# rsjahnige/CRYSTALS-Kyber

Hardware: AMD Instinct MI355X
Metric: ML-KEM-768 encaps+decaps/sec at batch 2^20; achieved HBM GB/s vs peak (higher is better)
Workload: dtype u32+f32 (64-bit Keccak lanes as 2 x u32; mod-3329 arithmetic exact on integers < 2^24 in the fp32 pipe; u8/u16 I/O)

## Files before the change

### crystals-kyber_amd/csrc/mlkem_kernels.hpp

```cpp
#pragma once
#include "mlkem_device.hpp"

namespace mlkem {

constexpr int WAVE = 64;

#ifndef MLKEM_KECCAK_MINWAVES
#define MLKEM_KECCAK_MINWAVES 6
#endif

struct MsgView {
    const uint8_t* p0; size_t stride0; unsigned len0;
    const uint8_t* p1; size_t stride1; unsigned len1;
};

__device__ __forceinline__ uint2 load_qword_tail(const uint8_t* p, unsigned avail) {
    if (avail >= 8) return *reinterpret_cast<const uint2*>(p);
    uint2 v;
    v.x = 0; v.y = 0;
    for (unsigned i = 0; i < avail; i++) {
        const uint32_t b = p[i];
        if (i < 4) v.x |= b << (8 * i);
        else v.y |= b << (8 * (i - 4));
    }
    return v;
}

#ifndef MLKEM_STAGE_ROWS
#define MLKEM_STAGE_ROWS 32
#endif
#ifndef MLKEM_STAGE_DMA
#define MLKEM_STAGE_DMA 1
#endif
constexpr int STAGE_ROWS = MLKEM_STAGE_ROWS;
constexpr int STAGE_GROUP = MLKEM_STAGE_DMA ? 2 : 7;
constexpr int STAGE_PARTS = WAVE / STAGE_ROWS;

template <int RATE>
__device__ __forceinline__ void wave_stage_block(uint2* stage, const MsgView& mv, size_t item0, size_t n_items, unsigned voff,
                                                 int part) {
    constexpr int NQ = RATE / 8, TOT = STAGE_ROWS * NQ, ITERS = (TOT + WAVE - 1) / WAVE;
    const unsigned l = (unsigned)lane_id(), total = mv.len0 + mv.len1;
#pragma unroll 1
    for (int it0 = 0; it0 < ITERS; it0 += STAGE_GROUP)
#pragma unroll
    for (int it = it0; it < it0 + STAGE_GROUP; it++) {
        if (it >= ITERS) break;
        const unsigned f = (unsigned)it * WAVE + l;
        if (TOT % WAVE != 0 && f >= (unsigned)TOT) break;
        const unsigned row = f / NQ, col = f - row * NQ;
        size_t item = item0 + (size_t)(part * STAGE_ROWS) + row;
        if (item >= n_items) item = n_items - 1;
        const unsigned pos = voff + 8u * col;
        uint2 v;
        v.x = 0; v.y = 0;
        if (pos < total) {
            if (pos < mv.len0) v = load_qword_tail(mv.p0 + item * mv.stride0 + pos, mv.len0 - pos);
            else v = load_qword_tail(mv.p1 + item * mv.stride1 + (pos - mv.len0), total - pos);
        }
        stage[f] = v;
    }
}

template <int RATE>
__device__ __forceinline__ void lane_xor_row(KeccakState& s, const uint2* stage, int part) {
    constexpr int NQ = RATE / 8;
    const int l = lane_id();
    if (l / STAGE_ROWS == part) {
        const uint2* row = stage + (l % STAGE_ROWS) * NQ;
#pragma unroll
        for (int w = 0; w < NQ; w++) {
            const uint2 v = row[w];
            s.lo[w] ^= v.x;
            s.hi[w] ^= v.y;
        }
    }
}
template <int RATE>
__device__ __forceinline__ void wave_absorb_block(KeccakState& s, uint2* stage, const MsgView& mv, size_t item0, size_t n_items,
                                                  unsigned voff) {
#pragma unroll 1
    for (int part = 0; part < STAGE_PARTS; part++) {
        wave_stage_block<RATE>(stage, mv, item0, n_items, voff, part);
        wave_lds_fence();
        lane_xor_row<RATE>(s, stage, part);
        wave_lds_fence();
    }
}

#ifndef MLKEM_STAGE_DMA
#define MLKEM_STAGE_DMA 1
#endif
template <int RATE>
struct DmaStage {
    static constexpr int NW = RATE / 4;
    static constexpr int NJ = (NW + 3) / 4;
    static constexpr int DWORDS = 2 * NJ * WAVE;
};

template <int RATE>
__device__ __forceinline__ void wave_dma_half(uint32_t* stage, const MsgView& mv, size_t item0, unsigned voff, unsigned valid,
                                              int half) {
    using D = DmaStage<RATE>;
    const unsigned l = (unsigned)lane_id_fresh(), rr = l >> 2, c4 = 4u * (l & 3u);
    const unsigned off0 = rr * (unsigned)mv.stride0 + c4, off1 = rr * (unsigned)mv.stride1 + c4;
    lds_dma_begin();
#pragma unroll
    for (int j = 0; j < D::NJ; j++) {
        const unsigned pos = 16u * (unsigned)j;
        const bool seg0 = voff + pos < mv.len0;
        const uint8_t* base = seg0 ? mv.p0 + (voff + pos) : mv.p1 + (voff + pos - mv.len0);
        const size_t stride = seg0 ? mv.stride0 : mv.stride1;
        const unsigned off = seg0 ? off0 : off1;
        if (pos + c4 < valid) {
#pragma unroll
            for (int g = 0; g < 2; g++)
                lds_dma_dword(base + (item0 + (size_t)(32 * half + 16 * g)) * stride, off, stage + (g * D::NJ + j) * WAVE);
        }
    }
}

template <int RATE, bool FULL>
__device__ __forceinline__ void lane_xor_dma(KeccakState& s, const uint32_t* stage, unsigned valid, int half) {
    using D = DmaStage<RATE>;
    const int l = lane_id_fresh();
    const uint32_t m = (l >> 5) == half ? 0xFFFFFFFFu : 0u;
    const uint32_t* row = stage + ((l >> 4) & 1) * (D::NJ * WAVE) + (l & 15) * 4;
#pragma unroll
    for (int j = 0; j < D::NJ; j++) {
        if (FULL || 16u * (unsigned)j < valid) {
            const uint4 v = *reinterpret_cast<const uint4*>(row + WAVE * j);
            const uint32_t d[4] = {v.x, v.y, v.z, v.w};
#pragma unroll
            for (int k = 0; k < 4; k++) {
                const int w = 4 * j + k;
                if (w < D::NW && (FULL || 4u * (unsigned)w < valid)) {
                    if (w & 1) s.hi[w >> 1] = __builtin_amdgcn_bitop3_b32(s.hi[w >> 1], d[k], m, 0x78);
                    else s.lo[w >> 1] = __builtin_amdgcn_bitop3_b32(s.lo[w >> 1], d[k], m, 0x78);
                }
            }
        }
    }
}
template <int NQ>
__device__ __forceinline__ void pin_state(KeccakState& s) {
#ifndef MLKEM_EMU
#pragma unroll
    for (int w = 0; w < NQ; w++) {
        asm volatile("" : "+v"(s.lo[w]));
        asm volatile("" : "+v"(s.hi[w]));
    }
#endif
}
template <int RATE, bool FULL>
__device__ __forceinline__ void wave_absorb_dma(KeccakState& s, uint32_t* st32, const MsgView& mv, size_t item0, unsigned voff,
                                                unsigned valid) {
    lds_dma_wait();
    wave_lds_fence();
    lane_xor_dma<RATE, FULL>(s, st32, valid, 0);
    pin_state<RATE / 8>(s);
    wave_lds_fence();
    wave_dma_half<RATE>(st32, mv, item0, voff, valid, 1);
    lds_dma_wait();
    wave_lds_fence();
    lane_xor_dma<RATE, FULL>(s, st32, valid, 1);
    pin_state<RATE / 8>(s);
    wave_lds_fence();
}

__device__ __forceinline__ void keccak_xor_byte_rt(KeccakState& s, unsigned pos, uint32_t byte) {
    const unsigned w = pos >> 2;
    const uint32_t v = byte << (8 * (pos & 3));
#define MLKEM_XB(W) keccak_word<W>(s) ^= (w == W) ? v : 0u;
    MLKEM_XB(0) MLKEM_XB(1) MLKEM_XB(2) MLKEM_XB(3) MLKEM_XB(4) MLKEM_XB(5) MLKEM_XB(6) MLKEM_XB(7)
    MLKEM_XB(8) MLKEM_XB(9) MLKEM_XB(10) MLKEM_XB(11) MLKEM_XB(12) MLKEM_XB(13) MLKEM_XB(14) MLKEM_XB(15)
    MLKEM_XB(16) MLKEM_XB(17) MLKEM_XB(18) MLKEM_XB(19) MLKEM_XB(20) MLKEM_XB(21) MLKEM_XB(22) MLKEM_XB(23)
    MLKEM_XB(24) MLKEM_XB(25) MLKEM_XB(26) MLKEM_XB(27) MLKEM_XB(28) MLKEM_XB(29) MLKEM_XB(30) MLKEM_XB(31)
    MLKEM_XB(32) MLKEM_XB(33) MLKEM_XB(34) MLKEM_XB(35) MLKEM_XB(36) MLKEM_XB(37) MLKEM_XB(38) MLKEM_XB(39)
    MLKEM_XB(40) MLKEM_XB(41)
#undef MLKEM_XB
}

template <int RATE, int SUFFIX>
__device__ __forceinline__ void wave_sponge_absorb(KeccakState& s, uint2* stage, const MsgView& mv, size_t item0,
                                                   size_t n_items) {
    const unsigned total = mv.len0 + mv.len1;
    keccak_zero(s);
#if MLKEM_STAGE_DMA
    if (item0 + WAVE <= n_items && total != 0 && total % 4 == 0 && (mv.len1 == 0 || mv.len0 % 16 == 0) &&
        mv.stride0 < (1u << 27) && mv.stride1 < (1u << 27)) {
        uint32_t* st32 = reinterpret_cast<uint32_t*>(stage);
        const unsigned nfull = total / (unsigned)RATE, rem = total - nfull * (unsigned)RATE;
        wave_dma_half<RATE>(st32, mv, item0, 0, nfull ? (unsigned)RATE : rem, 0);
#pragma unroll 1
        for (unsigned b = 0; b < nfull; b++) {
            wave_absorb_dma<RATE, true>(s, st32, mv, item0, b * RATE, RATE);
            if (b + 1 < nfull) wave_dma_half<RATE>(st32, mv, item0, (b + 1) * RATE, RATE, 0);
            else if (rem) wave_dma_half<RATE>(st32, mv, item0, nfull * RATE, rem, 0);
            keccak_f1600(s);
        }
        if (rem) wave_absorb_dma<RATE, false>(s, st32, mv, item0, nfull * RATE, rem);
        keccak_xor_byte_rt(s, rem, SUFFIX);
        keccak_xor_byte<RATE - 1>(s, 0x80);
        keccak_f1600(s);
        return;
    }
#endif
    unsigned voff = 0;
    while (total - voff >= (unsigned)RATE) {
        wave_absorb_block<RATE>(s, stage, mv, item0, n_items, voff);
        keccak_f1600(s);
        voff += RATE;
    }
    const unsigned rem = total - voff;
    if (rem) wave_absorb_block<RATE>(s, stage, mv, item0, n_items, voff);
    keccak_xor_byte_rt(s, rem, SUFFIX);
    keccak_xor_byte<RATE - 1>(s, 0x80);
    keccak_f1600(s);
}

constexpr int stage_qwords(int max_rate) {
    const int sync_q = STAGE_ROWS * (max_rate / 8);
    const int dma_q = MLKEM_STAGE_DMA ? 2 * ((max_rate / 4 + 3) / 4) * WAVE / 2 : 0;
    return sync_q > dma_q ? sync_q : dma_q;
}
constexpr int STAGE_QWORDS = stage_qwords(168);

__device__ __forceinline__ void store32(uint8_t* base, size_t stride, size_t item, const uint32_t (&w)[8]) {
    uint32_t* p = reinterpret_cast<uint32_t*>(base + item * stride);
#pragma unroll
    for (int i = 0; i < 8; i++) p[i] = w[i];
}
__device__ __forceinline__ void load32(const uint8_t* base, size_t stride, size_t item, uint32_t (&w)[8]) {
    const uint32_t* p = reinterpret_cast<const uint32_t*>(base + item * stride);
#pragma unroll
    for (int i = 0; i < 8; i++) w[i] = p[i];
}
#define MLKEM_STATE_WORDS8(s, FIRST, w)                                                             \
    {                                                                                               \
        w[0] = keccak_word<FIRST + 0>(s); w[1] = keccak_word<FIRST + 1>(s); w[2] = keccak_word<FIRST + 2>(s); \
        w[3] = keccak_word<FIRST + 3>(s); w[4] = keccak_word<FIRST + 4>(s); w[5] = keccak_word<FIRST + 5>(s); \
        w[6] = keccak_word<FIRST + 6>(s); w[7] = keccak_word<FIRST + 7>(s);                         \
    }
#define MLKEM_SET_WORDS8(s, FIRST, w)                                                               \
    {                                                                                               \
        keccak_word<FIRST + 0>(s) = w[0]; keccak_word<FIRST + 1>(s) = w[1]; keccak_word<FIRST + 2>(s) = w[2]; \
        keccak_word<FIRST + 3>(s) = w[3]; keccak_word<FIRST + 4>(s) = w[4]; keccak_word<FIRST + 5>(s) = w[5]; \
        keccak_word<FIRST + 6>(s) = w[6]; keccak_word<FIRST + 7>(s) = w[7];                         \
    }

__device__ __forceinline__ void lane_G64(KeccakState& s, const uint32_t (&x)[8], const uint32_t (&y)[8]) {
    keccak_zero(s);
    MLKEM_SET_WORDS8(s, 0, x)
    MLKEM_SET_WORDS8(s, 8, y)
    keccak_xor_byte<64>(s, 0x06);
    keccak_xor_byte<71>(s, 0x80);
    keccak_f1600(s);
}

template <int K>
__global__ void __launch_bounds__(WAVE, MLKEM_KECCAK_MINWAVES) k_hash_encaps(size_t n, const uint8_t* __restrict__ ek, const uint8_t* __restrict__ m,
                                                      uint8_t* __restrict__ Kout, uint8_t* __restrict__ r_ws) {
    __shared__ __attribute__((aligned(16))) uint2 stage[stage_qwords(136)];
    constexpr unsigned EK = 384 * K + 32;
    const size_t item0 = (size_t)blockIdx.x * WAVE, item = item0 + lane_id();
    KeccakState s;
    MsgView mv{ek, EK, EK, ek, EK, 0};
    wave_sponge_absorb<136, 0x06>(s, stage, mv, item0, n);
    uint32_t h[8], mm[8], w[8];
    MLKEM_STATE_WORDS8(s, 0, h)
    const size_t it = item < n ? item : n - 1;
    load32(m, 32, it, mm);
    lane_G64(s, mm, h);
    if (item < n) {
        MLKEM_STATE_WORDS8(s, 0, w)
        store32(Kout, 32, item, w);
        MLKEM_STATE_WORDS8(s, 8, w)
        store32(r_ws, 32, item, w);
    }
}

__global__ void __launch_bounds__(WAVE, MLKEM_KECCAK_MINWAVES) k_hash_g_shared(size_t n, const uint8_t* __restrict__ m, const uint8_t* __restrict__ h,
                                                                               uint8_t* __restrict__ Kout, uint8_t* __restrict__ r_ws) {
    const size_t item = (size_t)blockIdx.x * WAVE + lane_id();
    const size_t it = item < n ? item : n - 1;
    uint32_t mm[8], hh[8], w[8];
    load32(m, 32, it, mm);
    load32(h, 0, 0, hh);
    KeccakState s;
    lane_G64(s, mm, hh);
    if (item < n) {
        MLKEM_STATE_WORDS8(s, 0, w)
        store32(Kout, 32, item, w);
        MLKEM_STATE_WORDS8(s, 8, w)
        store32(r_ws, 32, item, w);
    }
}
__global__ void __launch_bounds__(256) k_status_fill(size_t n, const uint8_t* __restrict__ h_calc, const uint8_t* __restrict__ h_stored,
                                                     int32_t* __restrict__ status) {
    uint32_t diff = 0;
#pragma unroll
    for (int i = 0; i < 8; i++) diff |= reinterpret_cast<const uint32_t*>(h_calc)[i] ^ reinterpret_cast<const uint32_t*>(h_stored)[i];
    const int32_t v = diff ? -5 : 0;
    for (size_t i = (size_t)blockIdx.x * blockDim.x + threadIdx.x; i < n; i += (size_t)gridDim.x * blockDim.x) status[i] = v;
}
__global__ void __launch_bounds__(256) k_seed_split(size_t n, const uint4* __restrict__ seed, uint4* __restrict__ d, uint4* __restrict__ z) {
    const size_t g = (size_t)blockIdx.x * blockDim.x + threadIdx.x;
    if (g >= 4 * n) return;
    const size_t item = g >> 2;
    const unsigned part = (unsigned)(g & 3);
    const uint4 v = seed[g];
    if (part < 2) d[2 * item + part] = v;
    else z[2 * item + part - 2] = v;
}

template <int K, int CLEN, bool HASH_CHECK, int JRATE = 168>
__global__ void __launch_bounds__(WAVE, MLKEM_KECCAK_MINWAVES) k_hash_decaps(size_t n, const uint8_t* __restrict__ dk, const uint8_t* __restrict__ c,
                                                      const uint8_t* __restrict__ m_ws, uint8_t* __restrict__ Kp_ws,
                                                      uint8_t* __restrict__ r_ws, uint8_t* __restrict__ Kbar_ws,
                                                      int32_t* __restrict__ status, size_t dk_stride) {
    __shared__ __attribute__((aligned(16))) uint2 stage[STAGE_QWORDS];
    constexpr unsigned EK = 384 * K + 32;
    const size_t DK = dk_stride;
    const size_t nb = (n + WAVE - 1) / WAVE;
    const bool check_role = HASH_CHECK && blockIdx.x < nb;
    const size_t item0 = (size_t)(HASH_CHECK && !check_role ? blockIdx.x - nb : blockIdx.x) * WAVE;
    KeccakState s;
    uint32_t h[8], w[8];
    auto my_item = [&]() {
        const size_t i2 = item0 + (size_t)lane_id_fresh();
        return i2 < n ? i2 : n - 1;
    };
    if (check_role) {
        MsgView mv{dk + 384 * K, DK, EK, dk, DK, 0};
        wave_sponge_absorb<136, 0x06>(s, stage, mv, item0, n);
        MLKEM_STATE_WORDS8(s, 0, w)
        load32(dk + 768 * K + 32, DK, my_item(), h);
        uint32_t diff = 0;
#pragma unroll
        for (int i = 0; i < 8; i++) diff |= w[i] ^ h[i];
        const size_t i2 = item0 + (size_t)lane_id_fresh();
        if (i2 < n && status) status[i2] = diff ? -5 : 0;
        return;
    }
    {
        MsgView mv{dk + 768 * K + 64, DK, 32, c, CLEN, CLEN};
        wave_sponge_absorb<JRATE, 0x1F>(s, stage, mv, item0, n);
        const size_t i2 = item0 + (size_t)lane_id_fresh();
        if (i2 < n) {
            MLKEM_STATE_WORDS8(s, 0, w)
            store32(Kbar_ws, 32, i2, w);
        }
    }
    uint32_t mm[8];
    const size_t it = my_item();
    load32(m_ws, 32, it, mm);
    load32(dk + 768 * K + 32, DK, it, h);
    lane_G64(s, mm, h);
    const size_t item = item0 + (size_t)lane_id_fresh();
    if (item < n) {
        MLKEM_STATE_WORDS8(s, 0, w)
        store32(Kp_ws, 32, item, w);
        MLKEM_STATE_WORDS8(s, 8, w)
        store32(r_ws, 32, item, w);
        if (!HASH_CHECK && status) status[item] = 0;
    }
}

template <int K>
__global__ void __launch_bounds__(WAVE, MLKEM_KECCAK_MINWAVES) k_hash_keygen_seed(size_t n, const uint8_t* __restrict__ d, uint8_t* __restrict__ rho_ws,
                                                           uint8_t* __restrict__ sigma_ws) {
    const size_t item = (size_t)blockIdx.x * WAVE + lane_id();
    const size_t it = item < n ? item : n - 1;
    KeccakState s;
    uint32_t dd[8], w[8];
    load32(d, 32, it, dd);
    keccak_zero(s);
    MLKEM_SET_WORDS8(s, 0, dd)
    keccak_xor_byte<32>(s, (uint32_t)K);
    keccak_xor_byte<33>(s, 0x06);
    keccak_xor_byte<71>(s, 0x80);
    keccak_f1600(s);
    if (item < n) {
        MLKEM_STATE_WORDS8(s, 0, w)
        store32(rho_ws, 32, item, w);
        MLKEM_STATE_WORDS8(s, 8, w)
        store32(sigma_ws, 32, item, w);
    }
}

template <int K>
__global__ void __launch_bounds__(WAVE, MLKEM_KECCAK_MINWAVES) k_hash_keygen_fin(size_t n, const uint8_t* __restrict__ ek, const uint8_t* __restrict__ z,
                                                          uint8_t* __restrict__ dk) {
    __shared__ __attribute__((aligned(16))) uint2 stage[stage_qwords(136)];
    constexpr unsigned EK = 384 * K + 32, DK = 768 * K + 96;
    const size_t item0 = (size_t)blockIdx.x * WAVE, item = item0 + lane_id();
    KeccakState s;
    MsgView mv{ek, EK, EK, ek, EK, 0};
    wave_sponge_absorb<136, 0x06>(s, stage, mv, item0, n);
    if (item < n) {
        uint32_t w[8];
        MLKEM_STATE_WORDS8(s, 0, w)
        store32(dk + 768 * K + 32, DK, item, w);
        load32(z, 32, item, w);
        store32(dk + 768 * K + 64, DK, item, w);
    }
}

template <int KIND>
__global__ void __launch_bounds__(WAVE, 4) k_hash_batch(size_t n, const uint8_t* __restrict__ msg, unsigned len,
                                                                            size_t stride, uint8_t* __restrict__ out) {
    constexpr int RATE = KIND == 0 ? 136 : KIND == 1 ? 72 : 168;
    __shared__ __attribute__((aligned(16))) uint2 stage[stage_qwords(RATE)];
    const size_t item0 = (size_t)blockIdx.x * WAVE;
    KeccakState s;
    MsgView mv{msg, stride, len, msg, stride, 0};
    uint32_t w[8];
    wave_sponge_absorb<RATE, KIND == 2 ? 0x1F : 0x06>(s, stage, mv, item0, n);
    const size_t item = item0 + (size_t)lane_id_fresh();
    if (item < n) {
        MLKEM_STATE_WORDS8(s, 0, w)
        store32(out, KIND == 1 ? 64 : 32, item, w);
        if (KIND == 1) {
            MLKEM_STATE_WORDS8(s, 8, w)
            store32(out + 32, 64, item, w);
        }
    }
}

template <int RATE>
__global__ void __launch_bounds__(WAVE) k_sponge_raw(size_t n, const uint8_t* __restrict__ msg, unsigned nblocks, uint8_t* __restrict__ out,
                                                     unsigned outlen, size_t out_stride) {
    __shared__ __attribute__((aligned(16))) uint2 stage[STAGE_QWORDS];
    const size_t item0 = (size_t)blockIdx.x * WAVE, item = item0 + lane_id();
    KeccakState s;
    const unsigned total = nblocks * RATE;
    MsgView mv{msg, total, total, msg, total, 0};
    keccak_zero(s);
    for (unsigned voff = 0; voff < total; voff += RATE) {
        wave_absorb_block<RATE>(s, stage, mv, item0, n, voff);
        keccak_f1600(s);
    }
    uint8_t* o = out + (item < n ? item : n - 1) * out_stride;
    for (unsigned done = 0; done < outlen; done += RATE) {
        if (done) keccak_f1600(s);
        const unsigned take = outlen - done < (unsigned)RATE ? outlen - done : (unsigned)RATE;
        if (item < n) {
#define MLKEM_SQ(W)                                                                                         \
            if constexpr (W < RATE / 4) {                                                                   \
                if (4u * W + 4u <= take) *reinterpret_cast<uint32_t*>(o + done + 4 * W) = keccak_word<W>(s); \
                else if (4u * W < take) {                                                                   \
                    const uint32_t v = keccak_word<W>(s);                                                   \
                    for (unsigned b = 0; 4u * W + b < take; b++) o[done + 4 * W + b] = (uint8_t)(v >> (8 * b)); \
                }                                                                                           \
            }
            MLKEM_SQ(0) MLKEM_SQ(1) MLKEM_SQ(2) MLKEM_SQ(3) MLKEM_SQ(4) MLKEM_SQ(5) MLKEM_SQ(6) MLKEM_SQ(7)
            MLKEM_SQ(8) MLKEM_SQ(9) MLKEM_SQ(10) MLKEM_SQ(11) MLKEM_SQ(12) MLKEM_SQ(13) MLKEM_SQ(14) MLKEM_SQ(15)
            MLKEM_SQ(16) MLKEM_SQ(17) MLKEM_SQ(18) MLKEM_SQ(19) MLKEM_SQ(20) MLKEM_SQ(21) MLKEM_SQ(22) MLKEM_SQ(23)
            MLKEM_SQ(24) MLKEM_SQ(25) MLKEM_SQ(26) MLKEM_SQ(27) MLKEM_SQ(28) MLKEM_SQ(29) MLKEM_SQ(30) MLKEM_SQ(31)
            MLKEM_SQ(32) MLKEM_SQ(33) MLKEM_SQ(34) MLKEM_SQ(35) MLKEM_SQ(36) MLKEM_SQ(37) MLKEM_SQ(38) MLKEM_SQ(39)
            MLKEM_SQ(40) MLKEM_SQ(41)
#undef MLKEM_SQ
        }
    }
}

constexpr int RING = 128;
constexpr int RING_STRIDE = RING + 8;

constexpr int RESUME_WORDS = 52;
struct SampleArgs {
    size_t n_xof;
    const uint8_t* rho;
    size_t rho_stride;
    int K;
    int transpose;
    uint16_t* A;
    unsigned xof_blocks;
    size_t n_prf;
    const uint8_t* r;
    int per_item;
    int n_eta1;
    int eta1;
    uint8_t* prf;
    unsigned prf_stride;
    uint32_t* leftover;
    uint32_t* resume;
    uint32_t resume_cap;
    int list_mode;
    int prf_rate;
    uint8_t* retries;
};

template <class OutFn>
__device__ __forceinline__ void prf_eta3_tail(KeccakState& s, unsigned rate, OutFn out_of_lane, bool mine) {
    const unsigned nw = rate / 4;
    if (mine) {
        uint32_t* out = out_of_lane();
#define MLKEM_PT(W) if (W < nw) out[W] = keccak_word<W>(s);
        MLKEM_PT(32) MLKEM_PT(33) MLKEM_PT(34) MLKEM_PT(35) MLKEM_PT(36) MLKEM_PT(37) MLKEM_PT(38) MLKEM_PT(39) MLKEM_PT(40) MLKEM_PT(41)
#undef MLKEM_PT
    }
    keccak_f1600(s);
    if (mine) {
        uint32_t* out = out_of_lane() + nw;
#define MLKEM_PT(W) if (nw + W < 48u) out[W] = keccak_word<W>(s);
        MLKEM_PT(0) MLKEM_PT(1) MLKEM_PT(2) MLKEM_PT(3) MLKEM_PT(4) MLKEM_PT(5) MLKEM_PT(6) MLKEM_PT(7)
        MLKEM_PT(8) MLKEM_PT(9) MLKEM_PT(10) MLKEM_PT(11) MLKEM_PT(12) MLKEM_PT(13)
#undef MLKEM_PT
    }
}

__device__ __forceinline__ void ring_flush(const int16_t* ring, uint16_t* A, size_t g, bool valid, int cnt, int& flushed) {
    const int l = lane_id();
    const int has = (cnt - flushed >= 64) && valid;
    if (__ballot(has) == 0) return;
    const int grp = l >> 3, sub = l & 7;
#pragma unroll 1
    for (int step = 0; step < 8; step++) {
        const int p = step * 8 + grp;
        const int p_has = __shfl(has, p);
        const int p_flushed = __shfl(flushed, p);
        const size_t gp = (size_t)(uint32_t)__shfl((int)(uint32_t)g, p);
        if (p_has) {
            const int16_t* src = ring + p * RING_STRIDE + (p_flushed & (RING - 1)) + sub * 8;
            uint4 v = *reinterpret_cast<const uint4*>(src);
            *reinterpret_cast<uint4*>(A + gp * 256 + p_flushed + sub * 8) = v;
        }
    }
    if (has) flushed += 64;
}

constexpr int SAMPLE_CAP = 278;
constexpr int sample_nt5(int cap, int g) { return cap - 224 - 4 * g >= 4 ? 4 : (cap - 224 - 4 * g <= 0 ? 0 : cap - 224 - 4 * g); }

#define MLKEM_CAND(d)                                                      \
    {                                                                      \
        const bool ok = ((d) < (unsigned)QB) && (cnt < 256);               \
        if (ok) myring[cnt & (RING - 1)] = (int16_t)(d);                   \
        cnt += ok ? 1 : 0;                                                 \
    }
#define MLKEM_GROUP4(W0, NT)                                                                      \
    {                                                                                             \
        const uint32_t w0 = keccak_word<W0>(s), w1 = keccak_word<W0 + 1>(s), w2 = keccak_word<W0 + 2>(s); \
        const uint32_t v0 = w0 & 0xFFFFFFu, v1 = (w0 >> 24) | ((w1 & 0xFFFFu) << 8);              \
        const uint32_t v2 = (w1 >> 16) | ((w2 & 0xFFu) << 16), v3 = w2 >> 8;                      \
        if (NT > 0) { MLKEM_CAND(v0 & 0xFFFu) MLKEM_CAND(v0 >> 12) }                              \
        if (NT > 1) { MLKEM_CAND(v1 & 0xFFFu) MLKEM_CAND(v1 >> 12) }                              \
        if (NT > 2) { MLKEM_CAND(v2 & 0xFFFu) MLKEM_CAND(v2 >> 12) }                              \
        if (NT > 3) { MLKEM_CAND(v3 & 0xFFFu) MLKEM_CAND(v3 >> 12) }                              \
    }
#define MLKEM_GROUP4_CAP(W0, G)                                                                   \
    if constexpr (sample_nt5(CAP, G) == 4) { MLKEM_GROUP4(W0, 4) }                                \
    else { if (blk == 4) MLKEM_GROUP4(W0, sample_nt5(CAP, G)) else MLKEM_GROUP4(W0, 4) }

template <int QB = KQ, int CAP = SAMPLE_CAP>
__global__ void __launch_bounds__(WAVE) k_sample(SampleArgs a) {
    __shared__ __attribute__((aligned(16))) int16_t ring[WAVE * RING_STRIDE];
    const int l = lane_id();
    KeccakState s;
    if (blockIdx.x < a.xof_blocks) {
        const size_t limit = a.list_mode ? (size_t)a.leftover[0] : a.n_xof;
        const size_t stride = a.list_mode ? (size_t)gridDim.x * WAVE : ~(size_t)0 / 2;
      for (size_t base = (size_t)blockIdx.x * WAVE; base < limit; base += stride) {
        const size_t slot = base + l;
        const bool valid = slot < limit;
        const size_t slot_c = valid ? slot : limit - 1;
        const size_t g = a.list_mode ? (size_t)a.leftover[2 + slot_c] : slot_c;
        const size_t gc = g;
        uint32_t seed[8];
        unsigned i0, i1;
        if (a.K) {
            const size_t kk = (size_t)(a.K * a.K), item = gc / kk;
            const unsigned e = (unsigned)(gc - item * kk), ra = e / (unsigned)a.K, cb = e - ra * (unsigned)a.K;
            load32(a.rho, a.rho_stride, item, seed);
            i0 = a.transpose ? ra : cb;
            i1 = a.transpose ? cb : ra;
        } else {
            const uint8_t* sp = a.rho + gc * a.rho_stride;
#pragma unroll
            for (int i = 0; i < 8; i++)
                seed[i] = (uint32_t)sp[4 * i] | ((uint32_t)sp[4 * i + 1] << 8) | ((uint32_t)sp[4 * i + 2] << 16) |
                          ((uint32_t)sp[4 * i + 3] << 24);
            i0 = sp[32];
            i1 = sp[33];
        }
        int16_t* myring = ring + l * RING_STRIDE;
        unsigned nretry = 0;
        int cnt = 0, flushed = 0;
        bool fresh = true;
        int blk = 0;
        while (true) {
            if (fresh) {
                keccak_zero(s);
                MLKEM_SET_WORDS8(s, 0, seed)
                keccak_xor_byte<32>(s, i0 & 0xFFu);
                keccak_xor_byte<33>(s, i1 & 0xFFu);
                keccak_xor_byte<34>(s, 0x1F);
                keccak_xor_byte<167>(s, 0x80);
                cnt = 0; flushed = 0; blk = 0; fresh = false;
            }
            keccak_f1600(s);
            MLKEM_GROUP4_CAP(0, 0) MLKEM_GROUP4_CAP(3, 1) MLKEM_GROUP4_CAP(6, 2) MLKEM_GROUP4_CAP(9, 3)
            MLKEM_GROUP4_CAP(12, 4) MLKEM_GROUP4_CAP(15, 5) MLKEM_GROUP4_CAP(18, 6)
            wave_lds_fence();
            ring_flush(ring, a.A, g, valid, cnt, flushed);
            wave_lds_fence();
            MLKEM_GROUP4_CAP(21, 7) MLKEM_GROUP4_CAP(24, 8) MLKEM_GROUP4_CAP(27, 9) MLKEM_GROUP4_CAP(30, 10)
            MLKEM_GROUP4_CAP(33, 11) MLKEM_GROUP4_CAP(36, 12) MLKEM_GROUP4_CAP(39, 13)
            wave_lds_fence();
            ring_flush(ring, a.A, g, valid, cnt, flushed);
            wave_lds_fence();
            blk++;
            if (blk == 5 && cnt < 256) {
                i0 = (i0 + 1) & 0xFFu;
                i1 = (i1 + 1) & 0xFFu;
                fresh = true;
                nretry++;
            }
            if (__ballot(cnt < 256) == 0) break;
        }
        if (a.retries && valid && !a.list_mode) a.retries[g] = (uint8_t)(nretry < 255u ? nretry : 255u);
        wave_lds_fence();
      }
    } else {
        const size_t g = (size_t)(blockIdx.x - a.xof_blocks) * WAVE + l;
        const size_t gc = g < a.n_prf ? g : a.n_prf - 1;
        uint32_t seed[8];
        unsigned ctr, eta;
        if (a.per_item) {
            const size_t item = gc / (size_t)a.per_item;
            ctr = (unsigned)(gc - item * (size_t)a.per_item);
            load32(a.r, 32, item, seed);
            eta = (int)ctr < a.n_eta1 ? (unsigned)a.eta1 : 2u;
        } else {
            const uint8_t* sp = a.r + gc * 33;
#pragma unroll
            for (int i = 0; i < 8; i++)
                seed[i] = (uint32_t)sp[4 * i] | ((uint32_t)sp[4 * i + 1] << 8) | ((uint32_t)sp[4 * i + 2] << 16) |
                          ((uint32_t)sp[4 * i + 3] << 24);
            ctr = sp[32];
            eta = (unsigned)a.eta1;
        }
        keccak_zero(s);
        MLKEM_SET_WORDS8(s, 0, seed)
        keccak_xor_byte<32>(s, ctr & 0xFFu);
        keccak_xor_byte<33>(s, 0x1F);
        if (a.prf_rate == 136) keccak_xor_byte<135>(s, 0x80);
        else keccak_xor_byte<167>(s, 0x80);
        keccak_f1600(s);
        uint32_t* out = reinterpret_cast<uint32_t*>(a.prf + gc * a.prf_stride);
        if (g < a.n_prf) {
#define MLKEM_OW(W) out[W] = keccak_word<W>(s);
            MLKEM_OW(0) MLKEM_OW(1) MLKEM_OW(2) MLKEM_OW(3) MLKEM_OW(4) MLKEM_OW(5) MLKEM_OW(6) MLKEM_OW(7)
            MLKEM_OW(8) MLKEM_OW(9) MLKEM_OW(10) MLKEM_OW(11) MLKEM_OW(12) MLKEM_OW(13) MLKEM_OW(14) MLKEM_OW(15)
            MLKEM_OW(16) MLKEM_OW(17) MLKEM_OW(18) MLKEM_OW(19) MLKEM_OW(20) MLKEM_OW(21) MLKEM_OW(22) MLKEM_OW(23)
            MLKEM_OW(24) MLKEM_OW(25) MLKEM_OW(26) MLKEM_OW(27) MLKEM_OW(28) MLKEM_OW(29) MLKEM_OW(30) MLKEM_OW(31)
        }
#undef MLKEM_OW
        if (__ballot(eta == 3) != 0) {
            const bool mine = g < a.n_prf && eta == 3;
            auto out_fn = [out]() { return out; };
            prf_eta3_tail(s, a.prf_rate == 136 ? 136u : 168u, out_fn, mine);
        }
    }
}

}
```

### crystals-kyber_amd/csrc/mlkem_keyset.hpp

```cpp
#pragma once
#include "mlkem_pipeline.hpp"

namespace mlkem {

constexpr int32_t KS_ERR_ARG = -101;

struct KeysetView {
    const uint8_t* keys = nullptr;
    size_t key_stride = 0;
    size_t ek_off = 0;
    const uint8_t* h = nullptr;
    const uint16_t* At = nullptr;
    size_t n_keys = 0;
    bool has_dk = false;
};

struct KeysetLimits {
    size_t enc_max_k[3] = {1536, 1024, 768}, dec_max_k[3] = {3072, 2048, 3072};
    size_t enc_lat_k[3] = {256, 512, 256}, dec_lat_k[3] = {384, 256, 256};
    size_t enc_max(int k) const { return enc_max_k[k - 2]; }
    size_t dec_max(int k) const { return dec_max_k[k - 2]; }
    size_t enc_lat(int k) const { return enc_lat_k[k - 2]; }
    size_t dec_lat(int k) const { return dec_lat_k[k - 2]; }
    void set_all(size_t max_items, size_t lat_items) {
        for (int i = 0; i < 3; i++) {
            if (max_items != (size_t)-1) enc_max_k[i] = dec_max_k[i] = max_items;
            if (lat_items != (size_t)-1) enc_lat_k[i] = dec_lat_k[i] = lat_items;
        }
    }
};

__device__ __forceinline__ size_t keyset_key(const uint32_t* __restrict__ idx, size_t n_keys, size_t item) {
    if (!idx) return 0;
    const size_t k = idx[item];
    return k < n_keys ? k : 0;
}

__global__ void __launch_bounds__(WAVE, MLKEM_KECCAK_MINWAVES) k_hash_g_keyset(size_t n, const uint32_t* __restrict__ idx, size_t n_keys,
                                                                               const uint8_t* __restrict__ m, const uint8_t* __restrict__ hs,
                                                                               uint8_t* __restrict__ Kout, uint8_t* __restrict__ r_ws) {
    const size_t item = (size_t)blockIdx.x * WAVE + lane_id();
    const size_t it = item < n ? item : n - 1;
    uint32_t mm[8], hh[8], w[8];
    load32(m, 32, it, mm);
    load32(hs, 32, keyset_key(idx, n_keys, it), hh);
    KeccakState s;
    lane_G64(s, mm, hh);
    if (item < n) {
        MLKEM_STATE_WORDS8(s, 0, w)
        store32(Kout, 32, item, w);
        MLKEM_STATE_WORDS8(s, 8, w)
        store32(r_ws, 32, item, w);
    }
}

__global__ void __launch_bounds__(256) k_keyset_gather32(size_t n, const uint32_t* __restrict__ idx, size_t n_keys, const uint8_t* __restrict__ src,
                                                         size_t stride, uint32_t* __restrict__ dst) {
    const size_t g = (size_t)blockIdx.x * blockDim.x + threadIdx.x;
    if (g >= 8 * n) return;
    const size_t item = g >> 3;
    dst[g] = reinterpret_cast<const uint32_t*>(src + keyset_key(idx, n_keys, item) * stride)[g & 7];
}

template <int K, int CLEN, int JRATE>
__global__ void __launch_bounds__(WAVE, MLKEM_KECCAK_MINWAVES) k_hash_decaps_keyset(size_t n, const uint32_t* __restrict__ idx, size_t n_keys,
                                                                                    const uint8_t* __restrict__ hs, uint8_t* __restrict__ z_ws,
                                                                                    const uint8_t* __restrict__ c, const uint8_t* __restrict__ m_ws,
                                                                                    uint8_t* __restrict__ Kp_ws, uint8_t* __restrict__ r_ws,
                                                                                    uint8_t* __restrict__ Kbar_ws) {
    __shared__ __attribute__((aligned(16))) uint2 stage[STAGE_QWORDS];
    const size_t item0 = (size_t)blockIdx.x * WAVE;
    KeccakState s;
    uint32_t h[8], w[8];
    {
        MsgView mv{z_ws, 32, 32, c, CLEN, CLEN};
        wave_sponge_absorb<JRATE, 0x1F>(s, stage, mv, item0, n);
        const size_t i2 = item0 + (size_t)lane_id_fresh();
        if (i2 < n) {
            MLKEM_STATE_WORDS8(s, 0, w)
            store32(Kbar_ws, 32, i2, w);
            uint32_t* zr = reinterpret_cast<uint32_t*>(z_ws + i2 * 32);
#pragma unroll
            for (int q = 0; q < 8; q++) zr[q] = 0u;
        }
    }
    uint32_t mm[8];
    const size_t i3 = item0 + (size_t)lane_id_fresh(), it = i3 < n ? i3 : n - 1;
    load32(m_ws, 32, it, mm);
    load32(hs, 32, keyset_key(idx, n_keys, it), h);
    lane_G64(s, mm, h);
    const size_t item = item0 + (size_t)lane_id_fresh();
    if (item < n) {
        MLKEM_STATE_WORDS8(s, 0, w)
        store32(Kp_ws, 32, item, w);
        MLKEM_STATE_WORDS8(s, 8, w)
        store32(r_ws, 32, item, w);
    }
}

template <int K, int ETA1, int DU, int DV, bool COMPARE>
__global__ void __launch_bounds__(WAVE * KPKE2_WAVES, kpke2_minwaves(K))
k_encrypt2_keyset(size_t n, const uint32_t* __restrict__ idx, size_t n_keys, const uint8_t* __restrict__ ek, size_t ek_stride,
                  const uint16_t* __restrict__ At, const uint8_t* __restrict__ msg, const uint8_t* __restrict__ prf, uint8_t* __restrict__ c_out,
                  const uint8_t* __restrict__ c_in, const uint8_t* __restrict__ Kp, const uint8_t* __restrict__ Kbar, uint8_t* __restrict__ Kout) {
    __shared__ K2Lds<K + 1> lds_all[KPKE2_WAVES];
    const int wv = wave_id();
    const size_t item0 = 2 * ((size_t)blockIdx.x * KPKE2_WAVES + wv);
    if (item0 >= n) return;
    const size_t h = (size_t)(lane_id() >> 5), item = item0 + h < n ? item0 + h : item0;
    const size_t key = keyset_key(idx, n_keys, item);
    encrypt2_body<K, ETA1, DU, DV, COMPARE>(lds_all[wv].xch, item0, n, ek + key * ek_stride, 0, msg, At + key * (size_t)(K * K * 256), prf,
                                            c_out, c_in, Kp, Kbar, Kout, (int32_t*)nullptr, 0);
}

template <int K, int DU, int DV>
__global__ void __launch_bounds__(64 * KPKE4_WAVES, kpke4_minwaves(K)) k_decrypt4_keyset(size_t n, const uint32_t* __restrict__ idx, size_t n_keys,
                                                                                       const uint8_t* __restrict__ dk, size_t dk_stride,
                                                                                       const uint8_t* __restrict__ c, uint8_t* __restrict__ m_out) {
    const size_t quad = (size_t)blockIdx.x * KPKE4_WAVES + wave_id();
    if (4 * quad >= n) return;
    const size_t item_raw = 4 * quad + (size_t)rntt_lane().p, item = item_raw < n ? item_raw : n - 1;
    decrypt4_body<K, DU, DV>(quad, n, dk + keyset_key(idx, n_keys, item) * dk_stride, 0, c, m_out);
}

__global__ void __launch_bounds__(256) k_keyset_fix(size_t n, const uint32_t* __restrict__ idx, size_t n_keys, uint8_t* __restrict__ c,
                                                    unsigned c_len, uint8_t* __restrict__ Kout, int32_t* __restrict__ status) {
    for (size_t i = (size_t)blockIdx.x * blockDim.x + threadIdx.x; i < n; i += (size_t)gridDim.x * blockDim.x) {
        const bool bad = idx && (size_t)idx[i] >= n_keys;
        if (status) status[i] = bad ? KS_ERR_ARG : 0;
        if (!bad) continue;
        uint32_t* k = reinterpret_cast<uint32_t*>(Kout + i * 32);
        for (int w = 0; w < 8; w++) k[w] = 0;
        if (c) {
            uint32_t* cw = reinterpret_cast<uint32_t*>(c + i * c_len);
            for (unsigned w = 0; w < c_len / 4; w++) cw[w] = 0;
        }
    }
}

__global__ void __launch_bounds__(256) k_keyset_status_or(size_t n, const int32_t* __restrict__ status, uint32_t* __restrict__ out) {
    uint32_t v = 0;
    for (size_t i = (size_t)blockIdx.x * blockDim.x + threadIdx.x; i < n; i += (size_t)gridDim.x * blockDim.x) v |= (uint32_t)status[i];
    if (v) atomicOr(out, v);
}

template <int K, int ETA1>
struct __attribute__((aligned(16))) KeysetHand {
    uint8_t prf[(2 * K + 1) * (ETA1 == 3 ? 192 : 128)];
    uint8_t r[32], m[32], Kp[32], Kbar[32];
};

__device__ __forceinline__ void keyset_small_reject(size_t item, uint8_t* c, unsigned c_len, uint8_t* Kout, int32_t* status) {
    const unsigned l = (unsigned)lane_id();
    if (l < 8) reinterpret_cast<uint32_t*>(Kout + item * 32)[l] = 0;
    if (c)
        for (unsigned w = l; w < c_len / 4; w += WAVE) reinterpret_cast<uint32_t*>(c + item * c_len)[w] = 0;
    if (l == 0 && status) status[item] = KS_ERR_ARG;
}

template <int K, int ETA1, int DU, int DV, int NW>
__global__ void __launch_bounds__(WAVE * NW)
k_encaps_keyset_small(size_t n, const uint32_t* __restrict__ idx, size_t n_keys, const uint8_t* __restrict__ ek, size_t ek_stride,
                      const uint8_t* __restrict__ hs, const uint16_t* __restrict__ At, const uint8_t* __restrict__ m, uint8_t* __restrict__ c,
                      uint8_t* __restrict__ Kout, int32_t* __restrict__ status, int prf_rate) {
    __shared__ K2Lds<K + 1> xl;
    __shared__ KeysetHand<K, ETA1> hand;
    __shared__ uint2 rc_tables[NW][WK_RC_ENTRIES];
    __shared__ SmallSync sy;
    constexpr unsigned CLEN = 32 * (DU * K + DV);
    const int wv = wave_id();
    const size_t item = blockIdx.x;
    if (item >= n) return;
    const size_t key = idx ? (size_t)idx[item] : 0;
    if (key >= n_keys) {
        if (wv == 0) keyset_small_reject(item, c, CLEN, Kout, status);
        return;
    }
    const uint8_t* my_ek = ek + key * ek_stride;
    WkLane cst;
    wk_lane_init(cst, rc_tables[wave_id()]);
    if (threadIdx.x == 0) { sy.next_job = K * K; sy.jobs_done = 0; sy.r_ready = 0; sy.kbar_ready = 0; }
    block_barrier();
    if (wv == 0) {
        const int i = wk_index();
        uint2 v;
        v.x = 0; v.y = 0;
        if (i >= 0 && i < 4) v = reinterpret_cast<const uint2*>(m + item * 32)[i];
        else if (i >= 4 && i < 8) v = reinterpret_cast<const uint2*>(hs + key * 32)[i - 4];
        WkState a;
        a.lo = v.x; a.hi = v.y;
        if (i == 8) { a.lo = 0x06u; a.hi = 0x80000000u; }
        wk_permute(a, cst);
        uint2 o;
        o.x = a.lo; o.y = a.hi;
        if (wk_primary() && i < 4) reinterpret_cast<uint2*>(Kout + item * 32)[i] = o;
        else if (wk_primary() && i < 8) reinterpret_cast<uint2*>(hand.r)[i - 4] = o;
        flag_signal(&sy.r_ready);
    }
    small_jobs<K, ETA1>(sy, cst, nullptr, true, nullptr, hand.r, hand.prf, 2 * K + 1, (unsigned)prf_rate, nullptr);
    if (wv != 0) return;
    flag_wait(&sy.jobs_done, (uint32_t)(2 * K + 1));
    encrypt1_body<K, ETA1, DU, DV, false>(xl.xch, my_ek, m + item * 32, At + key * (size_t)(K * K * 256), hand.prf, c + item * CLEN, nullptr,
                                          nullptr, nullptr, nullptr, nullptr);
    if (lane_id() == 0 && status) status[item] = 0;
    wave_lds_fence();
    wave_zero_lds(hand);
    wave_zero_lds(xl);
#ifdef MLKEM_EMU_LDS_PROBE
    if (lane_id() == 0) { MLKEM_EMU_LDS_PROBE(&hand, sizeof hand); MLKEM_EMU_LDS_PROBE(&xl, sizeof xl); }
#endif
}

template <int K, int ETA1, int DU, int DV, int JRATE, int NW>
__global__ void __launch_bounds__(WAVE * NW)
k_decaps_keyset_small(size_t n, const uint32_t* __restrict__ idx, size_t n_keys, const uint8_t* __restrict__ dk, size_t dk_stride,
                      const uint8_t* __restrict__ hs, const uint16_t* __restrict__ At, const uint8_t* __restrict__ c, uint8_t* __restrict__ Kout,
                      int32_t* __restrict__ status, int prf_rate) {
    static_assert(NW >= 2, "roles of waves 0 and 1");
    __shared__ K2Lds<K + 1> xl;
    __shared__ KeysetHand<K, ETA1> hand;
    __shared__ uint2 rc_tables[NW][WK_RC_ENTRIES];
    __shared__ SmallSync sy;
    constexpr unsigned DK = 768 * K + 96, CLEN = 32 * (DU * K + DV);
    const int wv = wave_id();
    const size_t item = blockIdx.x;
    if (item >= n) return;
    const size_t key = idx ? (size_t)idx[item] : 0;
    if (key >= n_keys) {
        if (wv == 0) keyset_small_reject(item, nullptr, CLEN, Kout, status);
        return;
    }
    const uint8_t* my_dk = dk + key * dk_stride;
    const uint8_t* my_c = c + item * CLEN;
    WkLane cst;
    wk_lane_init(cst, rc_tables[wave_id()]);
    const int i = wk_index();
    const bool prim = wk_primary();
    if (threadIdx.x == 0) { sy.next_job = K * K; sy.jobs_done = 0; sy.r_ready = 0; sy.kbar_ready = 0; }
    block_barrier();
    if (wv == 0) {
        decrypt4_body<K, DU, DV>(0, 1, my_dk, (size_t)DK, my_c, hand.m);
        wave_global_fence();
        uint2 v;
        v.x = 0; v.y = 0;
        if (i >= 0 && i < 4) v = reinterpret_cast<const uint2*>(hand.m)[i];
        else if (i >= 4 && i < 8) v = reinterpret_cast<const uint2*>(hs + key * 32)[i - 4];
        WkState a;
        a.lo = v.x; a.hi = v.y;
        if (i == 8) { a.lo = 0x06u; a.hi = 0x80000000u; }
        wk_permute(a, cst);
        uint2 o;
        o.x = a.lo; o.y = a.hi;
        if (prim && i < 4) reinterpret_cast<uint2*>(hand.Kp)[i] = o;
        else if (prim && i < 8) reinterpret_cast<uint2*>(hand.r)[i - 4] = o;
        flag_signal(&sy.r_ready);
    } else if (wv == 1) {
        WkState a;
        wk_absorb<JRATE, 0x1F>(a, cst, my_dk + 768 * K + 64, 32, my_c, 32 + CLEN);
        uint2 o;
        o.x = a.lo; o.y = a.hi;
        if (prim && i < 4) reinterpret_cast<uint2*>(hand.Kbar)[i] = o;
        flag_signal(&sy.kbar_ready);
    }
    small_jobs<K, ETA1>(sy, cst, nullptr, true, nullptr, hand.r, hand.prf, 2 * K + 1, (unsigned)prf_rate, nullptr);
    if (wv != 0) return;
    flag_wait(&sy.jobs_done, (uint32_t)(2 * K + 1));
    encrypt1_body<K, ETA1, DU, DV, true>(xl.xch, my_dk + 384 * K, hand.m, At + key * (size_t)(K * K * 256), hand.prf, nullptr, my_c, hand.Kp,
                                         hand.Kbar, Kout + item * 32, nullptr, &sy.kbar_ready);
    if (lane_id() == 0 && status) status[item] = 0;
    wave_lds_fence();
    wave_zero_lds(hand);
    wave_zero_lds(xl);
#ifdef MLKEM_EMU_LDS_PROBE
    if (lane_id() == 0) { MLKEM_EMU_LDS_PROBE(&hand, sizeof hand); MLKEM_EMU_LDS_PROBE(&xl, sizeof xl); }
#endif
}

inline size_t keyset_table_bytes_per_key(const ParamSet& p, bool has_dk) {
    return (has_dk ? (size_t)p.dk_len : (size_t)p.ek_len) + 32 + (size_t)(p.k * p.k) * 512;
}

template <int K>
inline void keyset_import_run(stream_t st, const ParamSet& p, const KeysetView& ks, uint8_t* hs, uint16_t* At, int32_t* status,
                              uint32_t* status_or, const Workspace& ws) {
    const size_t n = ks.n_keys;
    zero_u32x2(st, status_or);
    if (status) {
        const uint8_t* ek = ks.has_dk ? nullptr : ks.keys;
        const uint8_t* dk = ks.has_dk ? ks.keys : nullptr;
        check_keys_dispatch(st, p.set, n, ek, dk, nullptr, nullptr, status, nullptr, min_sz(n, ws.cap), ws);
        launch("k_keyset_status_or", k_keyset_status_or, min_sz(ceil_div(n, 256), 1024), 256u, st, n, (const int32_t*)status, status_or);
    }
    hash_launch(st, 0, n, ks.keys + ks.ek_off, p.ek_len, ks.key_stride, hs);
    for (size_t c0 = 0; c0 < n; c0 += ws.cap) {
        const size_t cn = min_sz(ws.cap, n - c0);
        Workspace w = ws;
        w.A = At + c0 * (size_t)(K * K * 256);
        launch_sample_split(st, p, cn, 0, ks.keys + c0 * ks.key_stride + ks.ek_off + 384 * K, ks.key_stride, 1, nullptr, 0, 0, w);
    }
}

inline void keyset_seed_run(stream_t st, const ParamSet& p, size_t n, const uint8_t* seed, uint8_t* dk, uint8_t* tmp, const Workspace& ws) {
    uint8_t *d = tmp, *z = d + n * 32, *ek = z + n * 32;
    launch("k_seed_split", k_seed_split, ceil_div(4 * n, 256), 256, st, n, reinterpret_cast<const uint4*>(seed), reinterpret_cast<uint4*>(d),
           reinterpret_cast<uint4*>(z));
    keygen_dispatch(st, p.set, n, d, z, ek, dk, ws);
}

template <int K, int ETA1, int DU, int DV>
inline void encaps_keyset_run(stream_t st, const ParamSet& p, const KeysetView& ks, size_t n, const uint32_t* idx, const uint8_t* m, uint8_t* c,
                              uint8_t* Kout, int32_t* status, const Workspace& ws, const KeysetLimits& lim) {
    if (n == 0) return;
    const uint8_t* ek = ks.keys + ks.ek_off;
    if (n <= lim.enc_max(K)) {
        const int rate = ws.fips ? 136 : 168;
        if (n <= lim.enc_lat(K))
            launch("k_encaps_keyset_small", k_encaps_keyset_small<K, ETA1, DU, DV, SMALL_WAVES>, n, WAVE * SMALL_WAVES, st, n, idx, ks.n_keys, ek,
                   ks.key_stride, ks.h, ks.At, m, c, Kout, status, rate);
        else
            launch("k_encaps_keyset_small", k_encaps_keyset_small<K, ETA1, DU, DV, SMALL_WAVES_DENSE>, n, WAVE * SMALL_WAVES_DENSE, st, n, idx,
                   ks.n_keys, ek, ks.key_stride, ks.h, ks.At, m, c, Kout, status, rate);
        return;
    }
    for (size_t h0 = 0; h0 < n; h0 += ws.hcap) {
        const size_t hn = min_sz(ws.hcap, n - h0);
        const uint32_t* idh = idx ? idx + h0 : nullptr;
        launch("k_hash_g_keyset", k_hash_g_keyset, ceil_div(hn, WAVE), WAVE, st, hn, idh, ks.n_keys, m + h0 * 32, ks.h, Kout + h0 * 32, ws.r);
        for (size_t c0 = 0; c0 < hn; c0 += ws.cap) {
            const size_t cn = min_sz(ws.cap, hn - c0), i0 = h0 + c0;
            launch_sample_split(st, p, 0, cn, nullptr, 0, 1, ws.r + c0 * 32, 2 * K + 1, K, ws);
            launch("k_encrypt_keyset", k_encrypt2_keyset<K, ETA1, DU, DV, false>, ceil_div(ceil_div(cn, 2), KPKE2_WAVES), WAVE * KPKE2_WAVES, st, cn,
                   idx ? idx + i0 : nullptr, ks.n_keys, ek, ks.key_stride, ks.At, m + i0 * 32, (const uint8_t*)ws.prf, c + i0 * p.c_len,
                   (const uint8_t*)nullptr, (const uint8_t*)nullptr, (const uint8_t*)nullptr, (uint8_t*)nullptr);
        }
    }
    if (idx || status)
        launch("k_keyset_fix", k_keyset_fix, min_sz(ceil_div(n, 256), 1024), 256u, st, n, idx, ks.n_keys, c, p.c_len, Kout, status);
}

template <int K, int ETA1, int DU, int DV>
inline void decaps_keyset_run(stream_t st, const ParamSet& p, const KeysetView& ks, size_t n, const uint32_t* idx, const uint8_t* c,
                              uint8_t* Kout, int32_t* status, const Workspace& ws, const KeysetLimits& lim) {
    constexpr int CLEN = 32 * (DU * K + DV);
    if (n == 0) return;
    if (n <= lim.dec_max(K)) {
        const int rate = ws.fips ? 136 : 168;
#define MLKEM_DKS(JR, NW) launch("k_decaps_keyset_small", k_decaps_keyset_small<K, ETA1, DU, DV, JR, NW>, n, WAVE * NW, st, n, idx, ks.n_keys, \
                                 ks.keys, ks.key_stride, ks.h, ks.At, c, Kout, status, rate)
        if (!ws.fips && n <= lim.dec_lat(K)) MLKEM_DKS(168, SMALL_WAVES);
        else if (!ws.fips) MLKEM_DKS(168, SMALL_WAVES_DENSE);
        else if (n <= lim.dec_lat(K)) MLKEM_DKS(136, SMALL_WAVES);
        else MLKEM_DKS(136, SMALL_WAVES_DENSE);
#undef MLKEM_DKS
        return;
    }
    for (size_t h0 = 0; h0 < n; h0 += ws.hcap) {
        const size_t hn = min_sz(ws.hcap, n - h0);
        const uint32_t* idh = idx ? idx + h0 : nullptr;
        const uint8_t* ch = c + h0 * p.c_len;
        launch("k_decrypt_keyset", k_decrypt4_keyset<K, DU, DV>, ceil_div(ceil_div(hn, 4), KPKE4_WAVES), 64 * KPKE4_WAVES, st, hn, idh, ks.n_keys,
               ks.keys, ks.key_stride, ch, ws.m);
        launch("k_keyset_gather32", k_keyset_gather32, ceil_div(8 * hn, 256), 256u, st, hn, idh, ks.n_keys, ks.keys + 768 * K + 64, ks.key_stride,
               reinterpret_cast<uint32_t*>(ws.rho));
        if (!ws.fips)
            launch("k_hash_decaps_keyset", k_hash_decaps_keyset<K, CLEN, 168>, ceil_div(hn, WAVE), WAVE, st, hn, idh, ks.n_keys, ks.h,
                   ws.rho, ch, (const uint8_t*)ws.m, ws.Kp, ws.r, ws.Kbar);
        else
            launch("k_hash_decaps_keyset", k_hash_decaps_keyset<K, CLEN, 136>, ceil_div(hn, WAVE), WAVE, st, hn, idh, ks.n_keys, ks.h,
                   ws.rho, ch, (const uint8_t*)ws.m, ws.Kp, ws.r, ws.Kbar);
        for (size_t c0 = 0; c0 < hn; c0 += ws.cap) {
            const size_t cn = min_sz(ws.cap, hn - c0), i0 = h0 + c0;
            launch_sample_split(st, p, 0, cn, nullptr, 0, 1, ws.r + c0 * 32, 2 * K + 1, K, ws);
            launch("k_encrypt_cmp_keyset", k_encrypt2_keyset<K, ETA1, DU, DV, true>, ceil_div(ceil_div(cn, 2), KPKE2_WAVES), WAVE * KPKE2_WAVES, st,
                   cn, idx ? idx + i0 : nullptr, ks.n_keys, ks.keys + 384 * K, ks.key_stride, ks.At, (const uint8_t*)(ws.m + c0 * 32),
                   (const uint8_t*)ws.prf, (uint8_t*)nullptr, c + i0 * p.c_len, (const uint8_t*)(ws.Kp + c0 * 32), (const uint8_t*)(ws.Kbar + c0 * 32),
                   Kout + i0 * 32);
        }
    }
    if (idx || status)
        launch("k_keyset_fix", k_keyset_fix, min_sz(ceil_div(n, 256), 1024), 256u, st, n, idx, ks.n_keys, (uint8_t*)nullptr, p.c_len, Kout, status);
}

inline int keyset_import_dispatch(stream_t st, const ParamSet& p, const KeysetView& ks, uint8_t* hs, uint16_t* At, int32_t* status,
                                  uint32_t* status_or, const Workspace& ws) {
    switch (p.set) {
    case 512: keyset_import_run<2>(st, p, ks, hs, At, status, status_or, ws); break;
    case 768: keyset_import_run<3>(st, p, ks, hs, At, status, status_or, ws); break;
    default: keyset_import_run<4>(st, p, ks, hs, At, status, status_or, ws); break;
    }
    return 0;
}
inline int encaps_keyset_dispatch(stream_t st, const ParamSet& p, const KeysetView& ks, size_t n, const uint32_t* idx, const uint8_t* m,
                                  uint8_t* c, uint8_t* K, int32_t* status, const Workspace& ws, const KeysetLimits& lim) {
    switch (p.set) {
    case 512: encaps_keyset_run<2, 3, 10, 4>(st, p, ks, n, idx, m, c, K, status, ws, lim); break;
    case 768: encaps_keyset_run<3, 2, 10, 4>(st, p, ks, n, idx, m, c, K, status, ws, lim); break;
    default: encaps_keyset_run<4, 2, 11, 5>(st, p, ks, n, idx, m, c, K, status, ws, lim); break;
    }
    return 0;
}
inline int decaps_keyset_dispatch(stream_t st, const ParamSet& p, const KeysetView& ks, size_t n, const uint32_t* idx, const uint8_t* c,
                                  uint8_t* K, int32_t* status, const Workspace& ws, const KeysetLimits& lim) {
    switch (p.set) {
    case 512: decaps_keyset_run<2, 3, 10, 4>(st, p, ks, n, idx, c, K, status, ws, lim); break;
    case 768: decaps_keyset_run<3, 2, 10, 4>(st, p, ks, n, idx, c, K, status, ws, lim); break;
    default: decaps_keyset_run<4, 2, 11, 5>(st, p, ks, n, idx, c, K, status, ws, lim); break;
    }
    return 0;
}

}
```

### crystals-kyber_amd/csrc/mlkem_kpke2.hpp

```cpp
#pragma once
#include "mlkem_arith.hpp"
#include "mlkem_rntt.hpp"
#include <type_traits>

namespace mlkem {

#ifndef MLKEM_KPKE2_WAVES
#define MLKEM_KPKE2_WAVES 1
#endif
constexpr int KPKE2_WAVES = MLKEM_KPKE2_WAVES;
#ifdef MLKEM_KPKE2_MINWAVES
constexpr int kpke2_minwaves(int) { return MLKEM_KPKE2_MINWAVES; }
#else
constexpr int kpke2_minwaves(int k) { return k == 2 ? 4 : k == 3 ? 3 : 2; }
#endif

template <int NP>
struct __attribute__((aligned(16))) K2Lds {
    float2 xch[NP][2][128];
};

__device__ __forceinline__ int k2_slot(int pair) { return pair ^ ((pair & 64) ? 0x15 : 0) ^ ((pair & 32) ? 0x0A : 0); }
enum K2Layout { K2_LA = 0, K2_LB = 1, K2_LC = 2, K2_NAT = 3 };
__device__ __forceinline__ int k2_blk(int t) { return (((t >> 2) & 3) << 3) | ((t >> 4) << 2) | (t & 3); }
__device__ __forceinline__ int k2_lc_hi(int t) { return (((t >> 2) & 3) << 2) | ((t >> 4) << 1) | ((t >> 1) & 1); }
template <int LAYOUT>
__device__ __forceinline__ int k2_pair(int t, int j) {
    if constexpr (LAYOUT == K2_LA) return (j << 5) | t;
    else if constexpr (LAYOUT == K2_LB) return ((t >> 3) << 5) | (j << 3) | (t & 7);
    else if constexpr (LAYOUT == K2_LC) return (k2_lc_hi(t) << 3) | (j << 1) | (t & 1);
    else return (k2_blk(t) << 2) | j;
}
template <int LAYOUT>
__device__ __forceinline__ void k2_write(float2* xh, int t, const v2f (&p)[4]) {
#pragma unroll
    for (int j = 0; j < 4; j++) {
        float2 v;
        v.x = p[j].x; v.y = p[j].y;
        xh[k2_slot(k2_pair<LAYOUT>(t, j))] = v;
    }
}
template <int LAYOUT>
__device__ __forceinline__ void k2_read(const float2* xh, int t, v2f (&p)[4]) {
#pragma unroll
    for (int j = 0; j < 4; j++) {
        const float2 v = xh[k2_slot(k2_pair<LAYOUT>(t, j))];
        p[j] = v2f{v.x, v.y};
    }
}
template <int FROM, int TO, int NP>
__device__ __forceinline__ void k2_exchange(float2 (*xch)[2][128], int h, int t, v2f (&p)[NP][4]) {
#pragma unroll
    for (int q = 0; q < NP; q++) k2_write<FROM>(xch[q][h], t, p[q]);
    wave_lds_fence();
#pragma unroll
    for (int q = 0; q < NP; q++) k2_read<TO>(xch[q][h], t, p[q]);
    wave_lds_fence();
}

struct K2Tw {
    Tw b0, b1, b2, c0, c1, c2, d0, d1;
};
__device__ __forceinline__ void k2_twiddles_fwd(K2Tw& w, int t) {
    const Tw* z = ZETA_F.z;
    const int b = t >> 3, c = k2_lc_hi(t), n = k2_blk(t);
    w.b0 = z[4 + b]; w.b1 = z[8 + 2 * b]; w.b2 = z[9 + 2 * b];
    w.c0 = z[16 + c]; w.c1 = z[32 + 2 * c]; w.c2 = z[33 + 2 * c];
    w.d0 = z[64 + 2 * n]; w.d1 = z[65 + 2 * n];
}
__device__ __forceinline__ void k2_twiddles_inv(K2Tw& w, int t) {
    const Tw* z = ZETA_F.z;
    const int b = t >> 3, c = k2_lc_hi(t), n = k2_blk(t);
    w.d0 = z[127 - 2 * n]; w.d1 = z[126 - 2 * n];
    w.c1 = z[63 - 2 * c]; w.c2 = z[62 - 2 * c]; w.c0 = z[31 - c];
    w.b1 = z[15 - 2 * b]; w.b2 = z[14 - 2 * b]; w.b0 = z[7 - b];
}

template <int N>
__device__ __forceinline__ void k2_shoup_n(const Tw (&z)[N], v2f (&b)[N]) {
    v2f km[N], nk[N];
#pragma unroll
    for (int i = 0; i < N; i++) km[i] = fma2(b[i], splat2(z[i].zq), splat2(F_MAGIC));
#pragma unroll
    for (int i = 0; i < N; i++) nk[i] = fma2(km[i], splat2(-F_Q), splat2(F_MAGIC_Q));
#pragma unroll
    for (int i = 0; i < N; i++) b[i] = fma2(b[i], splat2(z[i].z), nk[i]);
}
template <int N>
__device__ __forceinline__ void k2_fred_n(v2f (&x)[N]) {
    v2f k[N];
#pragma unroll
    for (int i = 0; i < N; i++) k[i] = fma2(x[i], splat2(F_INVQ), splat2(F_MAGIC));
#pragma unroll
    for (int i = 0; i < N; i++) k[i] = k[i] - splat2(F_MAGIC);
#pragma unroll
    for (int i = 0; i < N; i++) x[i] = fma2(k[i], splat2(-F_Q), x[i]);
}
template <int N, bool GS>
__device__ __forceinline__ void k2_bfly_n(v2f (&a)[N], v2f (&b)[N], const Tw (&z)[N]) {
    if constexpr (!GS) {
        k2_shoup_n<N>(z, b);
#pragma unroll
        for (int i = 0; i < N; i++) { const v2f tt = b[i]; b[i] = a[i] - tt; a[i] = a[i] + tt; }
    } else {
        v2f d[N];
#pragma unroll
        for (int i = 0; i < N; i++) d[i] = b[i] - a[i];
#pragma unroll
        for (int i = 0; i < N; i++) a[i] = a[i] + b[i];
        k2_shoup_n<N>(z, d);
#pragma unroll
        for (int i = 0; i < N; i++) b[i] = d[i];
    }
}
template <int NP, bool GS>
__device__ __forceinline__ void k2_layer_hi(v2f (&p)[NP][4], Tw z) {
    v2f a[2 * NP], b[2 * NP];
    Tw zz[2 * NP];
#pragma unroll
    for (int q = 0; q < NP; q++) { a[2 * q] = p[q][0]; b[2 * q] = p[q][2]; a[2 * q + 1] = p[q][1]; b[2 * q + 1] = p[q][3]; zz[2 * q] = z; zz[2 * q + 1] = z; }
    k2_bfly_n<2 * NP, GS>(a, b, zz);
#pragma unroll
    for (int q = 0; q < NP; q++) { p[q][0] = a[2 * q]; p[q][2] = b[2 * q]; p[q][1] = a[2 * q + 1]; p[q][3] = b[2 * q + 1]; }
}
template <int NP, bool GS>
__device__ __forceinline__ void k2_layer_lo(v2f (&p)[NP][4], Tw z01, Tw z23) {
    v2f a[2 * NP], b[2 * NP];
    Tw zz[2 * NP];
#pragma unroll
    for (int q = 0; q < NP; q++) { a[2 * q] = p[q][0]; b[2 * q] = p[q][1]; a[2 * q + 1] = p[q][2]; b[2 * q + 1] = p[q][3]; zz[2 * q] = z01; zz[2 * q + 1] = z23; }
    k2_bfly_n<2 * NP, GS>(a, b, zz);
#pragma unroll
    for (int q = 0; q < NP; q++) { p[q][0] = a[2 * q]; p[q][1] = b[2 * q]; p[q][2] = a[2 * q + 1]; p[q][3] = b[2 * q + 1]; }
}
template <int NP, int R0, int R1>
__device__ __forceinline__ void k2_fred_pairs(v2f (&p)[NP][4]) {
    v2f x[2 * NP];
#pragma unroll
    for (int q = 0; q < NP; q++) { x[2 * q] = p[q][R0]; x[2 * q + 1] = p[q][R1]; }
    k2_fred_n<2 * NP>(x);
#pragma unroll
    for (int q = 0; q < NP; q++) { p[q][R0] = x[2 * q]; p[q][R1] = x[2 * q + 1]; }
}

template <int NP>
__device__ __forceinline__ void k2_ntt(v2f (&p)[NP][4], float2 (*xch)[2][128], int h, int t, const K2Tw& w) {
    k2_layer_hi<NP, false>(p, FZ1);
    k2_layer_lo<NP, false>(p, FZ2, FZ3);
    k2_exchange<K2_LA, K2_LB, NP>(xch, h, t, p);
    k2_layer_hi<NP, false>(p, w.b0);
    k2_layer_lo<NP, false>(p, w.b1, w.b2);
    k2_exchange<K2_LB, K2_LC, NP>(xch, h, t, p);
    k2_layer_hi<NP, false>(p, w.c0);
    k2_layer_lo<NP, false>(p, w.c1, w.c2);
    k2_exchange<K2_LC, K2_NAT, NP>(xch, h, t, p);
    k2_layer_lo<NP, false>(p, w.d0, w.d1);
}
template <int NP>
__device__ __forceinline__ void k2_intt(v2f (&p)[NP][4], float2 (*xch)[2][128], int h, int t, const K2Tw& w) {
    k2_layer_lo<NP, true>(p, w.d0, w.d1);
    k2_fred_pairs<NP, 0, 2>(p);
    k2_exchange<K2_NAT, K2_LC, NP>(xch, h, t, p);
    k2_layer_lo<NP, true>(p, w.c1, w.c2);
    k2_layer_hi<NP, true>(p, w.c0);
    k2_fred_pairs<NP, 0, 1>(p);
    k2_exchange<K2_LC, K2_LB, NP>(xch, h, t, p);
    k2_layer_lo<NP, true>(p, w.b1, w.b2);
    k2_layer_hi<NP, true>(p, w.b0);
    k2_fred_pairs<NP, 0, 1>(p);
    k2_exchange<K2_LB, K2_LA, NP>(xch, h, t, p);
    k2_layer_lo<NP, true>(p, FZ3, FZ2);
    {
        v2f sm[2 * NP], df[2 * NP];
        Tw zs[2 * NP], zd[2 * NP];
#pragma unroll
        for (int q = 0; q < NP; q++)
#pragma unroll
            for (int m = 0; m < 2; m++) {
                sm[2 * q + m] = p[q][m] + p[q][m + 2];
                df[2 * q + m] = p[q][m + 2] - p[q][m];
                zs[2 * q + m] = F_INV128; zd[2 * q + m] = F_INV128_Z1;
            }
        k2_shoup_n<2 * NP>(zs, sm);
        k2_shoup_n<2 * NP>(zd, df);
#pragma unroll
        for (int q = 0; q < NP; q++)
#pragma unroll
            for (int m = 0; m < 2; m++) { p[q][m] = sm[2 * q + m]; p[q][m + 2] = df[2 * q + m]; }
    }
    k2_exchange<K2_LA, K2_NAT, NP>(xch, h, t, p);
}

template <int ETA>
struct K2CbdRaw {
    uint32_t w[ETA == 2 ? 1 : 2];
};
template <int ETA>
__device__ __forceinline__ void k2_cbd_load_la(const uint8_t* prf, int t, K2CbdRaw<ETA>& r) {
    if constexpr (ETA == 2) {
        r.w[0] = (uint32_t)prf[t] | ((uint32_t)prf[t + 32] << 8) | ((uint32_t)prf[t + 64] << 16) | ((uint32_t)prf[t + 96] << 24);
    } else {
        uint32_t f[4];
#pragma unroll
        for (int j = 0; j < 4; j++) {
            const int o = ((3 * t) >> 1) + 48 * j;
            f[j] = (((uint32_t)prf[o] | ((uint32_t)prf[o + 1] << 8)) >> (4 * (t & 1))) & 0xFFFu;
        }
        r.w[0] = f[0] | (f[1] << 12);
        r.w[1] = f[2] | (f[3] << 12);
    }
}
__device__ __forceinline__ uint32_t k2_cbd_load_nat2(const uint8_t* prf, int t) { return reinterpret_cast<const uint32_t*>(prf)[t]; }
template <bool BIASED = false>
__device__ __forceinline__ void k2_cbd2_eval8(uint32_t t, v2f (&p)[4]) {
    const uint32_t s = (t & 0x55555555u) + ((t >> 1) & 0x55555555u);
    const uint32_t d = ((s & 0x33333333u) + 0x22222222u) - ((s >> 2) & 0x33333333u);
    const uint32_t lo = d & 0x0F0F0F0Fu, hi = (d >> 4) & 0x0F0F0F0Fu;
    float fl[4] = {(float)(lo & 0xFFu), (float)((lo >> 8) & 0xFFu), (float)((lo >> 16) & 0xFFu), (float)(lo >> 24)};
    float fh[4] = {(float)(hi & 0xFFu), (float)((hi >> 8) & 0xFFu), (float)((hi >> 16) & 0xFFu), (float)(hi >> 24)};
#ifndef MLKEM_EMU
    asm volatile("" : "+v"(fl[0]), "+v"(fl[1]), "+v"(fl[2]), "+v"(fl[3]), "+v"(fh[0]), "+v"(fh[1]), "+v"(fh[2]), "+v"(fh[3]));
#endif
#pragma unroll
    for (int j = 0; j < 4; j++) {
        if constexpr (BIASED) p[j] = v2f{fl[j], fh[j]};
        else p[j] = v2f{fl[j], fh[j]} - splat2(2.0f);
    }
}
template <int ETA>
__device__ __forceinline__ void k2_cbd_eval(const K2CbdRaw<ETA>& r, v2f (&p)[4]) {
    if constexpr (ETA == 2) {
        k2_cbd2_eval8<false>(r.w[0], p);
    } else {
        float a[4], b[4];
        cbd_eval_f<3>(r.w[0], a);
        cbd_eval_f<3>(r.w[1], b);
        p[0] = v2f{a[0], a[1]}; p[1] = v2f{a[2], a[3]}; p[2] = v2f{b[0], b[1]}; p[3] = v2f{b[2], b[3]};
    }
}

__device__ __forceinline__ void k2_gamma(const v2f (&y)[4], Tw d0, Tw d1, float (&yg)[4]) {
    yg[0] = fmulmod_shoup(d0, y[0].y);
    yg[1] = fmulmod_shoup(tw_neg(d0), y[1].y);
    yg[2] = fmulmod_shoup(d1, y[2].y);
    yg[3] = fmulmod_shoup(tw_neg(d1), y[3].y);
}
__device__ __forceinline__ void k2_basemul_acc(v2f (&acc)[4], const v2f (&a)[4], const v2f (&y)[4], const float (&yg)[4]) {
    v2f c[4];
#pragma unroll
    for (int j = 0; j < 4; j++) c[j] = fma2(splat2(a[j].x), y[j], acc[j]);
#pragma unroll
    for (int j = 0; j < 4; j++) {
        c[j].x = __builtin_fmaf(a[j].y, yg[j], c[j].x);
        c[j].y = __builtin_fmaf(a[j].y, y[j].x, c[j].y);
    }
    k2_fred_n<4>(c);
#pragma unroll
    for (int j = 0; j < 4; j++) acc[j] = c[j];
}

__device__ __forceinline__ void k2_unpack16(const uint4 v, v2f (&p)[4]) {
    const uint32_t w[4] = {v.x, v.y, v.z, v.w};
#pragma unroll
    for (int j = 0; j < 4; j++) p[j] = v2f{(float)(w[j] & 0xFFFFu), (float)(w[j] >> 16)};
}
__device__ __forceinline__ void k2_decode12(uint32_t w0, uint32_t w1, uint32_t w2, v2f (&p)[4]) {
    const uint32_t c0 = w0 & 0xFFFu, c1 = (w0 >> 12) & 0xFFFu, c2 = __builtin_amdgcn_alignbit(w1, w0, 24) & 0xFFFu, c3 = (w1 >> 4) & 0xFFFu;
    const uint32_t c4 = (w1 >> 16) & 0xFFFu, c5 = __builtin_amdgcn_alignbit(w2, w1, 28) & 0xFFFu, c6 = (w2 >> 8) & 0xFFFu, c7 = w2 >> 20;
    p[0] = v2f{(float)c0, (float)c1}; p[1] = v2f{(float)c2, (float)c3}; p[2] = v2f{(float)c4, (float)c5}; p[3] = v2f{(float)c6, (float)c7};
}

__device__ __forceinline__ uint32_t f_bits(float x) {
    union { float f; uint32_t u; } v;
    v.f = x;
    return v.u;
}
template <int D, bool BIASED = false>
__device__ __forceinline__ void k2_compress4(const v2f (&x)[4], unsigned (&c)[8]) {
    v2f tt[4], k0m[4], k0[4], r[4], km[4];
#pragma unroll
    for (int j = 0; j < 4; j++) tt[j] = fma2(x[j], splat2((float)(1 << D)), splat2(BIASED ? -(float)(2 << D) : 0.0f));
#pragma unroll
    for (int j = 0; j < 4; j++) k0m[j] = fma2(tt[j], splat2(F_INVQ), splat2(F_MAGIC));
#pragma unroll
    for (int j = 0; j < 4; j++) k0[j] = k0m[j] - splat2(F_MAGIC);
#pragma unroll
    for (int j = 0; j < 4; j++) r[j] = fma2(k0[j], splat2(-F_Q), tt[j]);
#pragma unroll
    for (int j = 0; j < 4; j++) km[j] = fma2(r[j], splat2(F_INVQ), splat2(F_MAGIC));
#pragma unroll
    for (int j = 0; j < 4; j++) {
        c[2 * j] = (f_bits(k0m[j].x) + f_bits(km[j].x)) & ((1u << D) - 1u);
        c[2 * j + 1] = (f_bits(k0m[j].y) + f_bits(km[j].y)) & ((1u << D) - 1u);
    }
}

__device__ __forceinline__ uint32_t k2_swap1(uint32_t v) {
#ifdef MLKEM_EMU
    return (uint32_t)emu_quad_shfl((int)v, (int)((threadIdx.x & 3) ^ 1));
#else
    return (uint32_t)__builtin_amdgcn_mov_dpp((int)v, 0xB1, 0xF, 0xF, true);
#endif
}
__device__ __forceinline__ uint32_t k2_prev_in_quad(uint32_t v) {
#ifdef MLKEM_EMU
    const int l = (int)(threadIdx.x & 3);
    return (uint32_t)emu_quad_shfl((int)v, l ? l - 1 : l);
#else
    return (uint32_t)__builtin_amdgcn_mov_dpp((int)v, 0x90, 0xF, 0xF, true);
#endif
}
__device__ __forceinline__ uint32_t k2_shl_hi(uint32_t hi, uint32_t lo, unsigned s) {
    return s ? __builtin_amdgcn_alignbit(hi, lo, 32u - s) : hi;
}

template <int D>
struct K2Piece {
    static_assert(D == 4 || D == 5 || D == 10 || D == 11 || D == 12, "ciphertext / key encodings of ML-KEM");
    static constexpr int NW = D == 4 ? 1 : D == 5 ? 2 : 3;
    uint32_t w[NW];
    static __device__ __forceinline__ int first(int t) {
        if constexpr (D == 4) return t;
        else if constexpr (D == 12) return 3 * t;
        else if constexpr (D == 10) return 5 * (t >> 1) + ((t & 1) ? 3 : 0);
        else if constexpr (D == 11) return 11 * (t >> 2) + ((88 * (t & 3)) >> 5);
        else return 5 * (t >> 2) + (t & 3);
    }
    static __device__ __forceinline__ int count(int t) {
        if constexpr (D == 4) return 1;
        else if constexpr (D == 12) return 3;
        else if constexpr (D == 10) return (t & 1) ? 2 : 3;
        else if constexpr (D == 11) return (t & 3) ? 3 : 2;
        else return (t & 3) == 3 ? 2 : 1;
    }
};
template <int D>
__device__ __forceinline__ void k2_encode(const unsigned (&c)[8], int t, K2Piece<D>& o) {
    if constexpr (D == 4) {
        o.w[0] = c[0] | (c[1] << 4) | (c[2] << 8) | (c[3] << 12) | (c[4] << 16) | (c[5] << 20) | (c[6] << 24) | (c[7] << 28);
    } else if constexpr (D == 12) {
        o.w[0] = c[0] | (c[1] << 12) | (c[2] << 24);
        o.w[1] = (c[2] >> 8) | (c[3] << 4) | (c[4] << 16) | (c[5] << 28);
        o.w[2] = (c[5] >> 4) | (c[6] << 8) | (c[7] << 20);
    } else if constexpr (D == 10) {
        const uint32_t v0 = c[0] | (c[1] << 10) | (c[2] << 20) | (c[3] << 30);
        const uint32_t v1 = (c[3] >> 2) | (c[4] << 8) | (c[5] << 18) | (c[6] << 28);
        const uint32_t v2 = (c[6] >> 4) | (c[7] << 6);
        const uint32_t other0 = k2_swap1(v0);
        const unsigned sh = (t & 1) ? 16u : 0u;
        o.w[0] = __builtin_amdgcn_alignbit(v1, v0, sh);
        o.w[1] = __builtin_amdgcn_alignbit(v2, v1, sh);
        o.w[2] = v2 | (other0 << 16);
    } else if constexpr (D == 11) {
        const uint32_t v0 = c[0] | (c[1] << 11) | (c[2] << 22);
        const uint32_t v1 = (c[2] >> 10) | (c[3] << 1) | (c[4] << 12) | (c[5] << 23);
        const uint32_t v2 = (c[5] >> 9) | (c[6] << 2) | (c[7] << 13);
        const int j = t & 3;
        const unsigned sh = (88u * (unsigned)j) & 31u;
        const uint32_t e0 = v0 << sh, e1 = k2_shl_hi(v1, v0, sh), e2 = k2_shl_hi(v2, v1, sh), e3 = k2_shl_hi(0u, v2, sh);
        const uint32_t tail = j == 0 ? e2 : e3;
        const uint32_t prev = k2_prev_in_quad(tail);
        o.w[0] = e0 | (j ? prev : 0u);
        o.w[1] = e1;
        o.w[2] = e2;
    } else {
        const uint32_t v0 = c[0] | (c[1] << 5) | (c[2] << 10) | (c[3] << 15) | (c[4] << 20) | (c[5] << 25) | (c[6] << 30);
        const uint32_t v1 = (c[6] >> 2) | (c[7] << 3);
        const int j = t & 3;
        const unsigned sh = 8u * (unsigned)j;
        const uint32_t e0 = v0 << sh, e1 = k2_shl_hi(v1, v0, sh);
        const uint32_t prev = k2_prev_in_quad(e1);
        o.w[0] = e0 | (j ? prev : 0u);
        o.w[1] = e1;
    }
}
template <int D>
__device__ __forceinline__ void k2_piece_load(const uint8_t* poly, int t, K2Piece<D>& o) {
    const uint32_t* g = reinterpret_cast<const uint32_t*>(poly) + K2Piece<D>::first(t);
#pragma unroll
    for (int i = 0; i < K2Piece<D>::NW; i++) o.w[i] = i < K2Piece<D>::count(t) ? stream_load4(g + i) : 0u;
}
template <int D>
__device__ __forceinline__ void k2_piece_store(uint8_t* poly, int t, const K2Piece<D>& o) {
    uint32_t* g = reinterpret_cast<uint32_t*>(poly) + K2Piece<D>::first(t);
#pragma unroll
    for (int i = 0; i < K2Piece<D>::NW; i++)
        if (i < K2Piece<D>::count(t)) g[i] = o.w[i];
}
template <int D>
__device__ __forceinline__ uint32_t k2_piece_diff(int t, const K2Piece<D>& a, const K2Piece<D>& ref) {
    uint32_t d = 0;
#pragma unroll
    for (int i = 0; i < K2Piece<D>::NW; i++)
        if (i < K2Piece<D>::count(t)) d |= a.w[i] ^ ref.w[i];
    return d;
}
template <int D, bool COMPARE, bool BIASED = false>
__device__ __forceinline__ uint32_t k2_emit(const v2f (&p)[4], int t, uint8_t* out, const K2Piece<D>& ref, bool store) {
    unsigned c[8];
    k2_compress4<D, BIASED>(p, c);
    K2Piece<D> o;
    k2_encode<D>(c, t, o);
    if constexpr (COMPARE) return k2_piece_diff<D>(t, o, ref);
    if (store) k2_piece_store<D>(out, t, o);
    return 0;
}

template <int K, int ETA1, int DU, int DV, bool COMPARE>
__device__ __forceinline__ void
encrypt2_body(float2 (*xch)[2][128], size_t item0, size_t n, const uint8_t* __restrict__ ek, size_t ek_stride, const uint8_t* __restrict__ msg,
              const uint16_t* __restrict__ A, const uint8_t* __restrict__ prf, uint8_t* __restrict__ c_out, const uint8_t* __restrict__ c_in,
              const uint8_t* __restrict__ Kp, const uint8_t* __restrict__ Kbar, uint8_t* __restrict__ Kout, int32_t* __restrict__ mod_status,
              size_t a_stride) {
    const int l = lane_id(), h = l >> 5, t = l & 31, nb = k2_blk(t);
    const bool valid = item0 + (size_t)h < n;
    const unsigned hh = valid ? (unsigned)h : 0u;
    constexpr unsigned PS = (ETA1 == 3) ? 192 : 128, CLEN = 32 * (DU * K + DV), PRFLEN = (2 * K + 1) * PS;
    const uint8_t* my_prf = prf + item0 * (size_t)PRFLEN + (size_t)(hh * PRFLEN);
    const uint8_t* my_ek = ek + item0 * ek_stride + (size_t)(hh * (unsigned)ek_stride);
    const uint16_t* my_A = A + item0 * a_stride + (size_t)(hh * (unsigned)a_stride);
    uint8_t* my_c = COMPARE ? nullptr : c_out + item0 * CLEN + (size_t)(hh * CLEN);
    const uint8_t* my_cin = COMPARE ? c_in + item0 * CLEN + (size_t)(hh * CLEN) : nullptr;
    const size_t item = item0 + hh;

    K2CbdRaw<ETA1> raw_y[K];
#pragma unroll
    for (int b = 0; b < K; b++) k2_cbd_load_la<ETA1>(my_prf + b * PS, t, raw_y[b]);
    uint4 a_all[K + 1][K];
#pragma unroll
    for (int a = 0; a < K; a++)
#pragma unroll
        for (int b = 0; b < K; b++) a_all[a][b] = *reinterpret_cast<const uint4*>(my_A + (a * K + b) * 256 + 8 * nb);
#pragma unroll
    for (int b = 0; b < K; b++) {
        const uint32_t* gp = reinterpret_cast<const uint32_t*>(my_ek + 384 * b) + 3 * nb;
        a_all[K][b].x = stream_load4(gp); a_all[K][b].y = stream_load4(gp + 1); a_all[K][b].z = stream_load4(gp + 2); a_all[K][b].w = 0u;
    }
    uint32_t raw_e[K + 1];
#pragma unroll
    for (int a = 0; a <= K; a++) raw_e[a] = k2_cbd_load_nat2(my_prf + (K + a) * PS, nb);
    const unsigned mb = msg[item * 32 + nb];

    v2f yh[K][4];
    float yg[K][4];
    {
        K2Tw tw;
        k2_twiddles_fwd(tw, t);
#pragma unroll
        for (int b = 0; b < K; b++) k2_cbd_eval<ETA1>(raw_y[b], yh[b]);
        k2_ntt<K>(yh, xch, h, t, tw);
#pragma unroll
        for (int b = 0; b < K; b++) {
            k2_fred_n<4>(yh[b]);
            k2_gamma(yh[b], tw.d0, tw.d1, yg[b]);
        }
    }
    uint32_t diff = 0;
    bool over = false;
    constexpr int NG = K + 1;
    v2f acc[NG][4];
    K2Piece<DU> cu_ref[NG];
    K2Piece<DV> cv_ref;
#pragma unroll
    for (int a = 0; a < NG; a++) {
#pragma unroll
        for (int j = 0; j < 4; j++) acc[a][j] = splat2(0.f);
#pragma unroll
        for (int b = 0; b < K; b++) {
            v2f av[4];
            if (a < K) {
                k2_unpack16(a_all[a][b], av);
            } else {
                k2_decode12(a_all[a][b].x, a_all[a][b].y, a_all[a][b].z, av);
#pragma unroll
                for (int j = 0; j < 4; j++) over = over || (av[j].x >= F_Q) || (av[j].y >= F_Q);
            }
            k2_basemul_acc(acc[a], av, yh[b], yg[b]);
        }
    }
    if constexpr (COMPARE) {
#pragma unroll
        for (int a = 0; a < NG; a++) {
            if (a < K) k2_piece_load<DU>(my_cin + a * 32 * DU, nb, cu_ref[a]);
            else k2_piece_load<DV>(my_cin + K * 32 * DU, nb, cv_ref);
        }
    }
    {
        K2Tw twi;
        k2_twiddles_inv(twi, t);
        k2_intt<NG>(acc, xch, h, t, twi);
    }
#pragma unroll
    for (int a = 0; a < NG; a++) {
        v2f e[4];
        k2_cbd2_eval8<true>(raw_e[a], e);
#pragma unroll
        for (int j = 0; j < 4; j++) acc[a][j] = acc[a][j] + e[j];
        if (a < K) {
            diff |= k2_emit<DU, COMPARE, true>(acc[a], nb, COMPARE ? nullptr : my_c + a * 32 * DU, cu_ref[a], valid);
        } else {
#pragma unroll
            for (int j = 0; j < 4; j++)
                acc[a][j] = acc[a][j] + v2f{((mb >> (2 * j)) & 1u) ? 1665.0f : 0.0f, ((mb >> (2 * j + 1)) & 1u) ? 1665.0f : 0.0f};
            diff |= k2_emit<DV, COMPARE, true>(acc[a], nb, COMPARE ? nullptr : my_c + K * 32 * DU, cv_ref, valid);
        }
    }
    if (mod_status) {
        const unsigned long long bal = __ballot(over);
        const bool bad = ((bal >> (32 * h)) & 0xFFFFFFFFull) != 0;
        if (t == 0 && valid) mod_status[item] = bad ? -4 : 0;
    }
    if constexpr (COMPARE) {
        const unsigned long long bal = __ballot(diff != 0);
        const uint32_t reject = ((bal >> (32 * h)) & 0xFFFFFFFFull) != 0 ? 0xFFFFFFFFu : 0u;
        if (t < 8 && valid) {
            const uint32_t kp = reinterpret_cast<const uint32_t*>(Kp + item * 32)[t];
            const uint32_t kb = reinterpret_cast<const uint32_t*>(Kbar + item * 32)[t];
            reinterpret_cast<uint32_t*>(Kout + item * 32)[t] = (kp & ~reject) | (kb & reject);
        }
    }
}
template <int K, int ETA1, int DU, int DV, bool COMPARE, bool A_T = false>
__device__ __forceinline__ void
encrypt1_body(float2 (*xch)[2][128], const uint8_t* __restrict__ ek, const uint8_t* __restrict__ msg, const uint16_t* __restrict__ A,
              const uint8_t* __restrict__ prf, uint8_t* __restrict__ c_out, const uint8_t* __restrict__ c_in, const uint8_t* __restrict__ Kp,
              const uint8_t* Kbar, uint8_t* __restrict__ Kout, int32_t* __restrict__ mod_status,
              const uint32_t* kbar_flag = nullptr) {
    const int l = lane_id(), h = l >> 5, t = l & 31, nb = k2_blk(t);
    constexpr unsigned PS = (ETA1 == 3) ? 192 : 128;
    constexpr int NG = K + 1, NL = (NG + 1) / 2;
    auto kind = [](int i) constexpr { return 2 * i + 1 < K ? 0 : (2 * i < K ? 1 : 2); };

    K2CbdRaw<ETA1> raw_y[K];
#pragma unroll
    for (int b = 0; b < K; b++) k2_cbd_load_la<ETA1>(prf + b * PS, t, raw_y[b]);
    uint4 a_all[NL][K];
    uint32_t raw_e[NL];
#pragma unroll
    for (int i = 0; i < NL; i++) {
        const int a = kind(i) == 2 ? K : 2 * i + h;
        const bool is_v = kind(i) == 2 || (kind(i) == 1 && h == 1);
#pragma unroll
        for (int b = 0; b < K; b++) {
            if (is_v) {
                const uint32_t* gp = reinterpret_cast<const uint32_t*>(ek + 384 * b) + 3 * nb;
                a_all[i][b].x = gp[0]; a_all[i][b].y = gp[1]; a_all[i][b].z = gp[2]; a_all[i][b].w = 0u;
            } else {
                a_all[i][b] = *reinterpret_cast<const uint4*>(A + (A_T ? b * K + a : a * K + b) * 256 + 8 * nb);
            }
        }
        raw_e[i] = k2_cbd_load_nat2(prf + (K + a) * PS, nb);
    }
    const unsigned mb = msg[nb];

    v2f yh[K][4];
    float yg[K][4];
    {
        K2Tw tw;
        k2_twiddles_fwd(tw, t);
#pragma unroll
        for (int b = 0; b < K; b++) k2_cbd_eval<ETA1>(raw_y[b], yh[b]);
        k2_ntt<K>(yh, xch, h, t, tw);
#pragma unroll
        for (int b = 0; b < K; b++) {
            k2_fred_n<4>(yh[b]);
            k2_gamma(yh[b], tw.d0, tw.d1, yg[b]);
        }
    }
    uint32_t diff = 0;
    bool over = false;
    v2f acc[NL][4];
    K2Piece<DU> cu_ref[NL];
    K2Piece<DV> cv_ref;
#pragma unroll
    for (int i = 0; i < NL; i++) {
        const bool is_v = kind(i) == 2 || (kind(i) == 1 && h == 1);
#pragma unroll
        for (int j = 0; j < 4; j++) acc[i][j] = splat2(0.f);
#pragma unroll
        for (int b = 0; b < K; b++) {
            v2f av[4];
            if (is_v) {
                k2_decode12(a_all[i][b].x, a_all[i][b].y, a_all[i][b].z, av);
#pragma unroll
                for (int j = 0; j < 4; j++) over = over || (av[j].x >= F_Q) || (av[j].y >= F_Q);
            } else {
                k2_unpack16(a_all[i][b], av);
            }
            k2_basemul_acc(acc[i], av, yh[b], yg[b]);
        }
    }
    if constexpr (COMPARE) {
#pragma unroll
        for (int i = 0; i < NL; i++) {
            const int a = kind(i) == 2 ? K : 2 * i + h;
            const bool is_v = kind(i) == 2 || (kind(i) == 1 && h == 1);
            if (is_v) k2_piece_load<DV>(c_in + K * 32 * DU, nb, cv_ref);
            else k2_piece_load<DU>(c_in + a * 32 * DU, nb, cu_ref[i]);
        }
    }
    {
        K2Tw twi;
        k2_twiddles_inv(twi, t);
        k2_intt<NL>(acc, xch, h, t, twi);
    }
#pragma unroll
    for (int i = 0; i < NL; i++) {
        const int a = kind(i) == 2 ? K : 2 * i + h;
        const bool is_v = kind(i) == 2 || (kind(i) == 1 && h == 1);
        const bool store = kind(i) != 2 || h == 0;
        v2f e[4];
        k2_cbd2_eval8<true>(raw_e[i], e);
#pragma unroll
        for (int j = 0; j < 4; j++) acc[i][j] = acc[i][j] + e[j];
        if (is_v) {
#pragma unroll
            for (int j = 0; j < 4; j++)
                acc[i][j] = acc[i][j] + v2f{((mb >> (2 * j)) & 1u) ? 1665.0f : 0.0f, ((mb >> (2 * j + 1)) & 1u) ? 1665.0f : 0.0f};
            diff |= k2_emit<DV, COMPARE, true>(acc[i], nb, COMPARE ? nullptr : c_out + K * 32 * DU, cv_ref, store);
        } else {
            diff |= k2_emit<DU, COMPARE, true>(acc[i], nb, COMPARE ? nullptr : c_out + a * 32 * DU, cu_ref[i], store);
        }
    }
    if (mod_status) {
        const bool bad = __ballot(over) != 0;
        if (l == 0) mod_status[0] = bad ? -4 : 0;
    }
    if constexpr (COMPARE) {
        const uint32_t reject = __ballot(diff != 0) != 0 ? 0xFFFFFFFFu : 0u;
        if (kbar_flag) flag_wait(kbar_flag, 1u);
        if (l < 8) {
            const uint32_t kp = reinterpret_cast<const uint32_t*>(Kp)[l];
            const uint32_t kb = reinterpret_cast<const uint32_t*>(Kbar)[l];
            reinterpret_cast<uint32_t*>(Kout)[l] = (kp & ~reject) | (kb & reject);
        }
    }
}

template <int K, int ETA1, int DU, int DV, bool COMPARE>
__global__ void __launch_bounds__(WAVE * KPKE2_WAVES, kpke2_minwaves(K))
k_encrypt2(size_t n, const uint8_t* __restrict__ ek, size_t ek_stride, const uint8_t* __restrict__ msg, const uint16_t* __restrict__ A,
           const uint8_t* __restrict__ prf, uint8_t* __restrict__ c_out, const uint8_t* __restrict__ c_in, const uint8_t* __restrict__ Kp,
           const uint8_t* __restrict__ Kbar, uint8_t* __restrict__ Kout, int32_t* __restrict__ mod_status, size_t a_stride) {
    __shared__ K2Lds<K + 1> lds_all[KPKE2_WAVES];
    const int wv = wave_id();
    const size_t item0 = 2 * ((size_t)blockIdx.x * KPKE2_WAVES + wv);
    if (item0 >= n) return;
    encrypt2_body<K, ETA1, DU, DV, COMPARE>(lds_all[wv].xch, item0, n, ek, ek_stride, msg, A, prf, c_out, c_in, Kp, Kbar, Kout, mod_status, a_stride);
}

__device__ __forceinline__ void k2_canon(const v2f (&p)[4], unsigned (&c)[8]) {
    v2f r[4] = {p[0], p[1], p[2], p[3]};
    k2_fred_n<4>(r);
#pragma unroll
    for (int j = 0; j < 4; j++) {
        const int a = (int)r[j].x, b = (int)r[j].y;
        c[2 * j] = (unsigned)(a + ((a >> 31) & KQ));
        c[2 * j + 1] = (unsigned)(b + ((b >> 31) & KQ));
    }
}

template <int K, int ETA1, bool KEM_DK>
__device__ __forceinline__ void
keygen2_body(float2 (*xch)[2][128], size_t item0, size_t n, const uint16_t* __restrict__ A, const uint8_t* __restrict__ prf,
             const uint8_t* __restrict__ rho, uint8_t* __restrict__ ek, uint8_t* __restrict__ dk) {
    const int l = lane_id(), h = l >> 5, t = l & 31, nb = k2_blk(t);
    const bool valid = item0 + (size_t)h < n;
    const unsigned hh = valid ? (unsigned)h : 0u;
    constexpr unsigned PS = (ETA1 == 3) ? 192 : 128, EK = 384 * K + 32, DK = KEM_DK ? 768 * K + 96 : 384 * K, PRFLEN = 2 * K * PS;
    const uint8_t* my_prf = prf + item0 * (size_t)PRFLEN + (size_t)(hh * PRFLEN);
    const uint16_t* my_A = A + item0 * (size_t)(K * K * 256) + (size_t)(hh * (unsigned)(K * K * 256));
    uint8_t* my_ek = ek + item0 * EK + (size_t)(hh * EK);
    uint8_t* my_dk = dk + item0 * DK + (size_t)(hh * DK);
    const size_t item = item0 + hh;

    K2CbdRaw<ETA1> raw_s[K], raw_e[K];
#pragma unroll
    for (int b = 0; b < K; b++) k2_cbd_load_la<ETA1>(my_prf + b * PS, t, raw_s[b]);
    constexpr bool PF = K >= 3;
    uint4 a_all[K][K];
    if constexpr (PF) {
#pragma unroll
        for (int a = 0; a < K; a++)
#pragma unroll
            for (int b = 0; b < K; b++) a_all[a][b] = *reinterpret_cast<const uint4*>(my_A + (a * K + b) * 256 + 8 * nb);
    }
#pragma unroll
    for (int a = 0; a < K; a++) k2_cbd_load_la<ETA1>(my_prf + (K + a) * PS, t, raw_e[a]);
    const uint32_t rho_w = reinterpret_cast<const uint32_t*>(rho + item * 32)[t & 7];
    K2Tw tw;
    k2_twiddles_fwd(tw, t);
    v2f sh[K][4];
    float sg[K][4];
#pragma unroll
    for (int b = 0; b < K; b++) k2_cbd_eval<ETA1>(raw_s[b], sh[b]);
    k2_ntt<K>(sh, xch, h, t, tw);
#pragma unroll
    for (int b = 0; b < K; b++) {
        k2_fred_n<4>(sh[b]);
        k2_gamma(sh[b], tw.d0, tw.d1, sg[b]);
        unsigned c[8];
        k2_canon(sh[b], c);
        K2Piece<12> o;
        k2_encode<12>(c, nb, o);
        if (valid) k2_piece_store<12>(my_dk + 384 * b, nb, o);
    }
    v2f eh[K][4];
#pragma unroll
    for (int a = 0; a < K; a++) k2_cbd_eval<ETA1>(raw_e[a], eh[a]);
    k2_ntt<K>(eh, xch, h, t, tw);
#pragma unroll
    for (int a = 0; a < K; a++) {
        v2f acc[4] = {splat2(0.f), splat2(0.f), splat2(0.f), splat2(0.f)};
#pragma unroll
        for (int b = 0; b < K; b++) {
            v2f av[4];
            if constexpr (!PF) a_all[a][b] = *reinterpret_cast<const uint4*>(my_A + (a * K + b) * 256 + 8 * nb);
            k2_unpack16(a_all[a][b], av);
            k2_basemul_acc(acc, av, sh[b], sg[b]);
        }
#pragma unroll
        for (int j = 0; j < 4; j++) acc[j] = acc[j] + eh[a][j];
        unsigned c[8];
        k2_canon(acc, c);
        K2Piece<12> o;
        k2_encode<12>(c, nb, o);
        if (valid) {
            k2_piece_store<12>(my_ek + 384 * a, nb, o);
            if constexpr (KEM_DK) k2_piece_store<12>(my_dk + 384 * K + 384 * a, nb, o);
        }
    }
    if (t < 8 && valid) {
        reinterpret_cast<uint32_t*>(my_ek + 384 * K)[t] = rho_w;
        if constexpr (KEM_DK) reinterpret_cast<uint32_t*>(my_dk + 768 * K)[t] = rho_w;
    }
}
template <int K, int ETA1, bool KEM_DK>
__global__ void __launch_bounds__(WAVE * KPKE2_WAVES, K == 2 ? kpke2_minwaves(2) : kpke2_minwaves(K + 1))
k_keygen2(size_t n, const uint16_t* __restrict__ A, const uint8_t* __restrict__ prf, const uint8_t* __restrict__ rho,
          uint8_t* __restrict__ ek, uint8_t* __restrict__ dk) {
    __shared__ K2Lds<K> lds_all[KPKE2_WAVES];
    const int wv = wave_id();
    const size_t item0 = 2 * ((size_t)blockIdx.x * KPKE2_WAVES + wv);
    if (item0 >= n) return;
    keygen2_body<K, ETA1, KEM_DK>(lds_all[wv].xch, item0, n, A, prf, rho, ek, dk);
}

}
```

### crystals-kyber_amd/csrc/mlkem_pipeline.hpp

```cpp
#pragma once
#include "mlkem_kernels.hpp"
#include "mlkem_sampler.hpp"
#include "mlkem_arith.hpp"
#include "mlkem_rntt.hpp"
#include "mlkem_kpke4.hpp"
#include "mlkem_kpke2.hpp"
#include "mlkem_wkeccak.hpp"
#include "mlkem_small.hpp"
#include "mlkem_sha3r.hpp"
#include "mlkem_check.hpp"
#include <stdlib.h>
#ifndef MLKEM_EMU
#include <vector>
#endif

namespace mlkem {

#ifdef MLKEM_EMU
using stream_t = void*;
#else
using stream_t = hipStream_t;
#endif

#ifndef MLKEM_EMU
struct LaunchRecorder {
    struct Rec { const char* label; hipEvent_t a, b; };
    std::vector<Rec> recs;
    bool failed = false;
};
inline LaunchRecorder*& launch_recorder() {
    static thread_local LaunchRecorder* r = nullptr;
    return r;
}
#endif

template <class... KArgs, class... Args>
inline void launch(const char* label, void (*kfn)(KArgs...), size_t grid, unsigned block, stream_t st, Args... args) {
    if (grid == 0) return;
#ifdef MLKEM_EMU
    (void)st; (void)label;
    emu::launch((unsigned)grid, block, [=] { kfn(args...); });
#else
    LaunchRecorder* rec = launch_recorder();
    LaunchRecorder::Rec r{label, nullptr, nullptr};
    bool timed = rec && hipEventCreate(&r.a) == hipSuccess && hipEventCreate(&r.b) == hipSuccess && hipEventRecord(r.a, st) == hipSuccess;
    kfn<<<dim3((unsigned)grid), dim3(block), 0, st>>>(args...);
    if (timed) timed = hipEventRecord(r.b, st) == hipSuccess;
    if (timed) {
        rec->recs.push_back(r);
    } else if (rec) {
        rec->failed = true;
        if (r.a) (void)hipEventDestroy(r.a);
        if (r.b) (void)hipEventDestroy(r.b);
    }
#endif
}

inline void zero_u32x2(stream_t st, uint32_t* p) {
#ifdef MLKEM_EMU
    (void)st;
    p[0] = 0; p[1] = 0;
#else
    (void)hipMemsetAsync(p, 0, 2 * sizeof(uint32_t), st);
#endif
}

struct ParamSet {
    int set, k, eta1, eta2, du, dv;
    unsigned ek_len, dk_len, c_len;
};
inline bool param_set(int set, ParamSet& p) {
    switch (set) {
    case 512: p = {512, 2, 3, 2, 10, 4, 0, 0, 0}; break;
    case 768: p = {768, 3, 2, 2, 10, 4, 0, 0, 0}; break;
    case 1024: p = {1024, 4, 2, 2, 11, 5, 0, 0, 0}; break;
    default: return false;
    }
    p.ek_len = 384u * p.k + 32;
    p.dk_len = 768u * p.k + 96;
    p.c_len = 32u * (p.du * p.k + p.dv);
    return true;
}

struct Workspace {
    uint16_t* A = nullptr;
    uint8_t *prf = nullptr, *r = nullptr, *rho = nullptr, *m = nullptr, *Kp = nullptr, *Kbar = nullptr;
    uint32_t* leftover = nullptr;
    uint32_t* resume = nullptr;
    uint32_t resume_cap = 0;
    size_t cap = 0;
    size_t hcap = 0;
    size_t wide_max = 2048;
    size_t wide_max_k[3] = {4096, 3072, 4096};
    size_t wide_kem(int k) const { return wide_max_k[k - 2]; }
    size_t small_max_k[3] = {1536, 768, 512};
    size_t small_max(int k) const { return small_max_k[k - 2]; }
    size_t small_lat_max = 256;
    size_t small_wide_max = 128;
    unsigned stages = 15;
    int fips = 0;
#ifndef MLKEM_EMU
    hipStream_t side = nullptr;
    hipEvent_t ev_fork = nullptr, ev_join = nullptr;
    bool side_on = true;
#endif
};
struct SideFork {
    stream_t main, side = nullptr;
#ifndef MLKEM_EMU
    hipEvent_t join = nullptr;
#endif
    SideFork(const Workspace& ws, stream_t st, size_t n) : main(st) {
#ifndef MLKEM_EMU
        if (ws.side && ws.side_on && n <= ws.cap && hipEventRecord(ws.ev_fork, st) == hipSuccess && hipStreamWaitEvent(ws.side, ws.ev_fork, 0) == hipSuccess) {
            side = ws.side;
            join = ws.ev_join;
        }
#else
        (void)ws; (void)n;
#endif
    }
    bool active() const { return side != nullptr; }
    stream_t xof_stream() const { return side ? side : main; }
    void join_main() {
#ifndef MLKEM_EMU
        if (side) {
            if (hipEventRecord(join, side) != hipSuccess || hipStreamWaitEvent(main, join, 0) != hipSuccess) (void)hipStreamSynchronize(side);
            side = nullptr;
        }
#endif
    }
};

inline size_t ceil_div(size_t a, size_t b) { return (a + b - 1) / b; }
inline size_t min_sz(size_t a, size_t b) { return a < b ? a : b; }

template <int QB = KQ, int CAP = SAMPLE_CAP>
inline void launch_sample_split(stream_t st, const ParamSet& p, size_t n_xof_items, size_t n_prf_items, const uint8_t* rho, size_t rho_stride,
                                int transpose, const uint8_t* r, int prf_per_item, int n_eta1, const Workspace& ws) {
    SampleArgs a{};
    a.n_xof = n_xof_items * (size_t)(p.k * p.k);
    a.rho = rho; a.rho_stride = rho_stride; a.K = p.k; a.transpose = transpose; a.A = ws.A;
    a.xof_blocks = (unsigned)ceil_div(a.n_xof, WAVE);
    a.n_prf = n_prf_items * (size_t)prf_per_item;
    a.r = r; a.per_item = prf_per_item; a.n_eta1 = n_eta1; a.eta1 = p.eta1; a.prf = ws.prf;
    a.prf_stride = p.eta1 == 3 ? 192 : 128;
    a.leftover = ws.leftover;
    a.resume = ws.resume;
    a.resume_cap = ws.resume ? ws.resume_cap : 0;
    a.list_mode = 0;
    a.prf_rate = ws.fips ? 136 : 168;
    const size_t grid = a.xof_blocks + ceil_div(a.n_prf, WAVE);
    if (grid == 0) return;
    if (n_xof_items <= ws.wide_kem(p.k) && n_prf_items <= ws.wide_kem(p.k)) {
        launch("k_sample_direct", k_sample<QB, CAP>, grid, WAVE, st, a);
        return;
    }
    if (a.n_xof) zero_u32x2(st, ws.leftover);
    launch("k_sample_main", k_sample_main<QB>, grid, WAVE, st, a);
    if (a.n_xof == 0) return;
    SampleArgs t = a;
    t.list_mode = 1;
    t.n_prf = 0;
    t.xof_blocks = (unsigned)(ceil_div(a.n_xof, WAVE * 16) + 1);
    if (a.resume_cap) {
        launch("k_sample_tail", k_sample_resume<QB, CAP>, (size_t)t.xof_blocks, WAVE, st, t);
        t.xof_blocks = (unsigned)(ceil_div(a.n_xof, WAVE * 256) + 1);
    }
    launch("k_sample_restart", k_sample<QB, CAP>, (size_t)t.xof_blocks, WAVE, st, t);
}
template <int QB = KQ, int CAP = SAMPLE_CAP>
inline void launch_sample(stream_t st, const ParamSet& p, size_t n, const uint8_t* rho, size_t rho_stride, int transpose,
                          const uint8_t* r, int prf_per_item, int n_eta1, const Workspace& ws) {
    launch_sample_split<QB, CAP>(st, p, n, n, rho, rho_stride, transpose, r, prf_per_item, n_eta1, ws);
}

template <int K, int ETA1, int DU, int DV, bool CMP, class... Args>
inline void encrypt_launch(const char* label, stream_t st, size_t n, Args... args) {
    launch(label, k_encrypt2<K, ETA1, DU, DV, CMP>, ceil_div(ceil_div(n, 2), KPKE2_WAVES), WAVE * KPKE2_WAVES, st, n, args...);
}

template <int K, int ETA1>
inline void keygen_run(stream_t st, const ParamSet& p, size_t n, const uint8_t* d, const uint8_t* z, uint8_t* ek, uint8_t* dk,
                       const Workspace& ws) {
    const bool kem = z != nullptr;
    const size_t dk_len = kem ? (size_t)p.dk_len : (size_t)(384 * K);
    if (n && n <= ws.small_max(K)) {
        const int rate = ws.fips ? 136 : 168;
#define MLKEM_KS(KEM, NW) launch("k_keygen_small", k_keygen_small<K, ETA1, KEM, NW>, n, WAVE * NW, st, n, d, z, ek, dk, rate)
        const bool lat = n <= ws.small_lat_max;
        if (kem && lat) MLKEM_KS(true, SMALL_WAVES);
        else if (kem) MLKEM_KS(true, SMALL_WAVES_DENSE);
        else if (lat) MLKEM_KS(false, SMALL_WAVES);
        else MLKEM_KS(false, SMALL_WAVES_DENSE);
#undef MLKEM_KS
        return;
    }
    for (size_t h0 = 0; h0 < n; h0 += ws.hcap) {
        const size_t hn = min_sz(ws.hcap, n - h0);
        launch("k_hash_keygen_seed", k_hash_keygen_seed<K>, ceil_div(hn, WAVE), WAVE, st, hn, d + h0 * 32, ws.rho, ws.r);
        for (size_t c0 = 0; c0 < hn; c0 += ws.cap) {
            const size_t cn = min_sz(ws.cap, hn - c0), i0 = h0 + c0;
            launch_sample(st, p, cn, ws.rho + c0 * 32, 32, 0, ws.r + c0 * 32, 2 * K, 2 * K, ws);
            const size_t kgrid = ceil_div(ceil_div(cn, 2), KPKE2_WAVES);
            if (kem)
                launch("k_keygen", k_keygen2<K, ETA1, true>, kgrid, WAVE * KPKE2_WAVES, st, cn, (const uint16_t*)ws.A, (const uint8_t*)ws.prf,
                       (const uint8_t*)(ws.rho + c0 * 32), ek + i0 * p.ek_len, dk + i0 * dk_len);
            else
                launch("k_keygen", k_keygen2<K, ETA1, false>, kgrid, WAVE * KPKE2_WAVES, st, cn, (const uint16_t*)ws.A, (const uint8_t*)ws.prf,
                       (const uint8_t*)(ws.rho + c0 * 32), ek + i0 * p.ek_len, dk + i0 * dk_len);
        }
        if (kem && n <= ws.wide_kem(K))
            launch("k_hash_keygen_fin", k_hash_keygen_fin_w<K>, hn, WAVE, st, hn, (const uint8_t*)(ek + h0 * p.ek_len), z + h0 * 32, dk + h0 * p.dk_len);
        else if (kem)
            launch("k_hash_keygen_fin", k_hash_keygen_fin<K>, ceil_div(hn, WAVE), WAVE, st, hn, (const uint8_t*)(ek + h0 * p.ek_len),
                   z + h0 * 32, dk + h0 * p.dk_len);
    }
}

template <int K, int ETA1, int DU, int DV>
inline void encaps_run(stream_t st, const ParamSet& p, size_t n, const uint8_t* ek, const uint8_t* m, uint8_t* c, uint8_t* Kout,
                       int32_t* mod_status, const Workspace& ws, const uint8_t* r_user = nullptr) {
    if (n == 0) return;
    if (!r_user && n <= ws.small_max(K)) {
        const int rate = ws.fips ? 136 : 168;
        if (n <= ws.small_lat_max)
            launch("k_encaps_small", k_encaps_small<K, ETA1, DU, DV, SMALL_WAVES>, n, WAVE * SMALL_WAVES, st, n, ek, m, c, Kout, mod_status, rate);
        else
            launch("k_encaps_small", k_encaps_small<K, ETA1, DU, DV, SMALL_WAVES_DENSE>, n, WAVE * SMALL_WAVES_DENSE, st, n, ek, m, c, Kout, mod_status, rate);
        return;
    }
    SideFork fork(ws, st, r_user ? (size_t)-1 : n);
    if (fork.active()) launch_sample_split(fork.xof_stream(), p, n, 0, ek + 384 * K, p.ek_len, 1, nullptr, 2 * K + 1, K, ws);
    for (size_t h0 = 0; h0 < n; h0 += ws.hcap) {
        const size_t hn = min_sz(ws.hcap, n - h0);
        const uint8_t* r_h = r_user ? r_user + h0 * 32 : (const uint8_t*)ws.r;
        if (!(ws.stages & 1u)) {
        } else if (!r_user && n <= ws.wide_kem(K))
            launch("k_hash_encaps", k_hash_encaps_w<K>, hn, WAVE, st, hn, ek + h0 * p.ek_len, m + h0 * 32, Kout + h0 * 32, ws.r);
        else if (!r_user)
            launch("k_hash_encaps", k_hash_encaps<K>, ceil_div(hn, WAVE), WAVE, st, hn, ek + h0 * p.ek_len, m + h0 * 32, Kout + h0 * 32, ws.r);
        for (size_t c0 = 0; c0 < hn; c0 += ws.cap) {
            const size_t cn = min_sz(ws.cap, hn - c0), i0 = h0 + c0;
            const uint8_t* eki = ek + i0 * p.ek_len;
            if (fork.active()) {
                launch_sample_split(st, p, 0, cn, nullptr, 0, 1, r_h + c0 * 32, 2 * K + 1, K, ws);
                fork.join_main();
            } else if (ws.stages & 2u) {
                launch_sample(st, p, cn, eki + 384 * K, p.ek_len, 1, r_h + c0 * 32, 2 * K + 1, K, ws);
            }
            if (ws.stages & 4u)
            encrypt_launch<K, ETA1, DU, DV, false>("k_encrypt", st, cn, eki, (size_t)p.ek_len, m + i0 * 32, (const uint16_t*)ws.A, (const uint8_t*)ws.prf,
                   c + i0 * p.c_len, (const uint8_t*)nullptr, (const uint8_t*)nullptr, (const uint8_t*)nullptr, (uint8_t*)nullptr,
                   mod_status ? mod_status + i0 : (int32_t*)nullptr, (size_t)(K * K * 256));
        }
    }
}

template <int K, int DU, int DV>
inline void decrypt_launch(stream_t st, size_t n, const uint8_t* dk, size_t dk_stride, const uint8_t* c, uint8_t* m) {
    launch("k_decrypt", k_decrypt4<K, DU, DV>, ceil_div(ceil_div(n, 4), KPKE4_WAVES), 64 * KPKE4_WAVES, st, n, dk, dk_stride, c, m);
}

template <int K, int ETA1, int DU, int DV>
inline void decaps_run(stream_t st, const ParamSet& p, size_t n, const uint8_t* dk, const uint8_t* c, uint8_t* Kout,
                       int32_t* status, bool hash_check, const Workspace& ws) {
    constexpr int CLEN = 32 * (DU * K + DV);
    if (n && n <= ws.small_max(K)) {
        const int rate = ws.fips ? 136 : 168;
        int32_t* sts = hash_check ? status : (int32_t*)nullptr;
#define MLKEM_DS(HC, JR, NW) launch("k_decaps_small", k_decaps_small<K, ETA1, DU, DV, HC, JR, NW>, (HC) ? 2 * n : n, WAVE * NW, st, n, dk, c, Kout, sts, rate)
        constexpr int LW = K >= 3 ? SMALL_WAVES_WIDE : SMALL_WAVES;
#define MLKEM_DS2(HC, JR) do { if (n <= ws.small_wide_max) MLKEM_DS(HC, JR, LW); else if (n <= ws.small_lat_max) MLKEM_DS(HC, JR, SMALL_WAVES); else MLKEM_DS(HC, JR, SMALL_WAVES_DENSE); } while (0)
        if (hash_check && !ws.fips) MLKEM_DS2(true, 168);
        else if (!ws.fips) MLKEM_DS2(false, 168);
        else if (hash_check) MLKEM_DS2(true, 136);
        else MLKEM_DS2(false, 136);
#undef MLKEM_DS2
#undef MLKEM_DS
        return;
    }
    for (size_t h0 = 0; h0 < n; h0 += ws.hcap) {
        const size_t hn = min_sz(ws.hcap, n - h0);
        const uint8_t* dkh = dk + h0 * p.dk_len;
        const uint8_t* ch = c + h0 * p.c_len;
        SideFork fork(ws, st, n);
        if (fork.active()) launch_sample_split(fork.xof_stream(), p, n, 0, dk + 768 * K, p.dk_len, 1, nullptr, 2 * K + 1, K, ws);
        if (ws.stages & 8u) decrypt_launch<K, DU, DV>(st, hn, dkh, (size_t)p.dk_len, ch, ws.m);
        int32_t* sth = (hash_check && status) ? status + h0 : (int32_t*)nullptr;
        const size_t hgrid = ceil_div(hn, WAVE);
        if (!(ws.stages & 1u)) {
        } else if (n <= ws.wide_kem(K)) {
            if (hash_check && !ws.fips)
                launch("k_hash_decaps", k_hash_decaps_w<K, CLEN, true, 168>, 2 * hn, WAVE, st, hn, dkh, ch, (const uint8_t*)ws.m, ws.Kp, ws.r, ws.Kbar, sth, (size_t)p.dk_len);
            else if (!ws.fips)
                launch("k_hash_decaps", k_hash_decaps_w<K, CLEN, false, 168>, hn, WAVE, st, hn, dkh, ch, (const uint8_t*)ws.m, ws.Kp, ws.r, ws.Kbar, sth, (size_t)p.dk_len);
            else if (hash_check)
                launch("k_hash_decaps", k_hash_decaps_w<K, CLEN, true, 136>, 2 * hn, WAVE, st, hn, dkh, ch, (const uint8_t*)ws.m, ws.Kp, ws.r, ws.Kbar, sth, (size_t)p.dk_len);
            else
                launch("k_hash_decaps", k_hash_decaps_w<K, CLEN, false, 136>, hn, WAVE, st, hn, dkh, ch, (const uint8_t*)ws.m, ws.Kp, ws.r, ws.Kbar, sth, (size_t)p.dk_len);
        } else
        if (hash_check && !ws.fips)
            launch("k_hash_decaps", k_hash_decaps<K, CLEN, true, 168>, 2 * hgrid, WAVE, st, hn, dkh, ch, (const uint8_t*)ws.m, ws.Kp, ws.r, ws.Kbar, sth, (size_t)p.dk_len);
        else if (!ws.fips)
            launch("k_hash_decaps", k_hash_decaps<K, CLEN, false, 168>, hgrid, WAVE, st, hn, dkh, ch, (const uint8_t*)ws.m, ws.Kp, ws.r, ws.Kbar, sth, (size_t)p.dk_len);
        else if (hash_check)
            launch("k_hash_decaps", k_hash_decaps<K, CLEN, true, 136>, 2 * hgrid, WAVE, st, hn, dkh, ch, (const uint8_t*)ws.m, ws.Kp, ws.r, ws.Kbar, sth, (size_t)p.dk_len);
        else
            launch("k_hash_decaps", k_hash_decaps<K, CLEN, false, 136>, hgrid, WAVE, st, hn, dkh, ch, (const uint8_t*)ws.m, ws.Kp, ws.r, ws.Kbar, sth, (size_t)p.dk_len);
        for (size_t c0 = 0; c0 < hn; c0 += ws.cap) {
            const size_t cn = min_sz(ws.cap, hn - c0), i0 = h0 + c0;
            const uint8_t* dki = dk + i0 * p.dk_len;
            if (fork.active()) {
                launch_sample_split(st, p, 0, cn, nullptr, 0, 1, ws.r + c0 * 32, 2 * K + 1, K, ws);
                fork.join_main();
            } else if (ws.stages & 2u) {
                launch_sample(st, p, cn, dki + 768 * K, p.dk_len, 1, ws.r + c0 * 32, 2 * K + 1, K, ws);
            }
            if (ws.stages & 4u)
            encrypt_launch<K, ETA1, DU, DV, true>("k_encrypt_cmp", st, cn, dki + 384 * K, (size_t)p.dk_len, (const uint8_t*)(ws.m + c0 * 32), (const uint16_t*)ws.A,
                   (const uint8_t*)ws.prf, (uint8_t*)nullptr, c + i0 * p.c_len, (const uint8_t*)(ws.Kp + c0 * 32),
                   (const uint8_t*)(ws.Kbar + c0 * 32), Kout + i0 * 32, (int32_t*)nullptr, (size_t)(K * K * 256));
        }
    }
}

inline size_t seed_stage_bytes(const ParamSet& p) { return 64 + (size_t)p.ek_len + (size_t)p.dk_len; }
template <int K, int ETA1, int DU, int DV>
inline void decaps_seed_run(stream_t st, const ParamSet& p, size_t n, const uint8_t* seed, const uint8_t* c, uint8_t* Kout, uint8_t* stage,
                            size_t stage_items, const Workspace& ws) {
    if (n == 0) return;
    if (n <= ws.small_max(K)) {
        const int rate = ws.fips ? 136 : 168;
#define MLKEM_DSS(JR, NW) launch("k_decaps_seed_small", k_decaps_seed_small<K, ETA1, DU, DV, JR, NW>, n, WAVE * NW, st, n, seed, c, Kout, rate)
#define MLKEM_DSS2(JR) do { if (n <= ws.small_lat_max) MLKEM_DSS(JR, SMALL_WAVES); else MLKEM_DSS(JR, SMALL_WAVES_DENSE); } while (0)
        if (!ws.fips) MLKEM_DSS2(168);
        else MLKEM_DSS2(136);
#undef MLKEM_DSS2
#undef MLKEM_DSS
        return;
    }
    for (size_t s0 = 0; s0 < n; s0 += stage_items) {
        const size_t sn = min_sz(stage_items, n - s0);
        uint8_t *d = stage, *z = d + stage_items * 32, *ek = z + stage_items * 32, *dk = ek + stage_items * p.ek_len;
        launch("k_seed_split", k_seed_split, ceil_div(4 * sn, 256), 256, st, sn, reinterpret_cast<const uint4*>(seed + s0 * 64),
               reinterpret_cast<uint4*>(d), reinterpret_cast<uint4*>(z));
        keygen_run<K, ETA1>(st, p, sn, d, z, ek, dk, ws);
        decaps_run<K, ETA1, DU, DV>(st, p, sn, dk, c + s0 * p.c_len, Kout + s0 * 32, nullptr, false, ws);
    }
}

inline size_t check_stage_bytes(const ParamSet& p, bool has_ek, bool seed, bool pct) {
    return (seed ? seed_stage_bytes(p) : 0) + (pct ? (size_t)p.c_len + 64 + (has_ek ? 0 : (size_t)p.ek_len) : 0);
}
inline size_t check_chunk_items(const ParamSet& p, size_t n, bool has_ek, bool seed, bool pct, size_t stage_bytes, const Workspace& ws) {
    const size_t need = check_stage_bytes(p, has_ek, seed, pct);
    size_t c = min_sz(n, ws.cap);
    if (need) c = min_sz(c, stage_bytes / need);
    return c ? c : 1;
}
template <int K, int ETA1, int DU, int DV>
inline void check_keys_run(stream_t st, const ParamSet& p, size_t n, const uint8_t* ek, const uint8_t* dk, const uint8_t* seed,
                           const uint8_t* m, int32_t* status, uint8_t* stage, size_t chunk, const Workspace& ws) {
    if (n == 0) return;
    const bool hash_in = n <= ws.wide_kem(K);
    for (size_t s0 = 0; s0 < n; s0 += chunk) {
        const size_t sn = min_sz(chunk, n - s0);
        const uint8_t* eki = ek ? ek + s0 * p.ek_len : nullptr;
        const uint8_t* dki = dk ? dk + s0 * p.dk_len : nullptr;
        const uint8_t *sek = nullptr, *sdk = nullptr, *Kc = nullptr, *Kd = nullptr;
        uint8_t* q = stage;
        if (seed) {
            uint8_t *d = q, *z = d + chunk * 32, *e2 = z + chunk * 32, *d2 = e2 + chunk * p.ek_len;
            q = d2 + chunk * p.dk_len;
            launch("k_seed_split", k_seed_split, ceil_div(4 * sn, 256), 256, st, sn, reinterpret_cast<const uint4*>(seed + s0 * 64),
                   reinterpret_cast<uint4*>(d), reinterpret_cast<uint4*>(z));
            keygen_run<K, ETA1>(st, p, sn, d, z, e2, d2, ws);
            sek = e2;
            sdk = d2;
        }
        if (m) {
            const uint8_t* pek = eki;
            if (!ek) {
                uint8_t* g = q;
                q += chunk * p.ek_len;
                launch("k_gather_rows", k_gather_rows, ceil_div(sn * (p.ek_len / 16), 256), 256, st, sn, dki + 384 * K, (size_t)p.dk_len, g,
                       (unsigned)p.ek_len);
                pek = g;
            }
            uint8_t *c = q, *kc = c + chunk * p.c_len, *kd = kc + chunk * 32;
            encaps_run<K, ETA1, DU, DV>(st, p, sn, pek, m + s0 * 32, c, kc, nullptr, ws);
            decaps_run<K, ETA1, DU, DV>(st, p, sn, dki, c, kd, nullptr, false, ws);
            Kc = kc;
            Kd = kd;
        }
        if (hash_in) {
            launch("k_check_keys", k_check_keys<K, true>, sn, 2 * WAVE, st, sn, eki, dki, (const uint8_t*)nullptr, sek, sdk, Kc, Kd, status + s0);
        } else {
            if (dki) launch("k_hash_batch", k_hash_batch<0>, ceil_div(sn, WAVE), WAVE, st, sn, dki + 384 * K, (unsigned)p.ek_len, (size_t)p.dk_len, ws.Kp);
            launch("k_check_keys", k_check_keys<K, false>, ceil_div(sn, 4), WAVE * 4, st, sn, eki, dki, (const uint8_t*)ws.Kp, sek, sdk, Kc, Kd,
                   status + s0);
        }
    }
}

template <int K, int ETA1, int DU, int DV>
inline void encaps_shared_run(stream_t st, const ParamSet& p, size_t n, const uint8_t* ek, const uint8_t* m, uint8_t* c, uint8_t* Kout,
                              const Workspace& ws) {
    const Workspace& w = ws;
    uint8_t* h = ws.rho;
    launch("k_hash_batch", k_hash_batch<0>, (size_t)1, WAVE, st, (size_t)1, ek, (unsigned)p.ek_len, (size_t)p.ek_len, h);
    launch_sample_split(st, p, 1, 0, ek + 384 * K, p.ek_len, 1, nullptr, 0, 0, w);
    for (size_t h0 = 0; h0 < n; h0 += ws.hcap) {
        const size_t hn = min_sz(ws.hcap, n - h0);
        launch("k_hash_g_shared", k_hash_g_shared, ceil_div(hn, WAVE), WAVE, st, hn, m + h0 * 32, (const uint8_t*)h, Kout + h0 * 32, ws.r);
        for (size_t c0 = 0; c0 < hn; c0 += ws.cap) {
            const size_t cn = min_sz(ws.cap, hn - c0), i0 = h0 + c0;
            launch_sample_split(st, p, 0, cn, nullptr, 0, 1, ws.r + c0 * 32, 2 * K + 1, K, w);
            encrypt_launch<K, ETA1, DU, DV, false>("k_encrypt", st, cn, ek, (size_t)0,
                   m + i0 * 32, (const uint16_t*)w.A, (const uint8_t*)w.prf, c + i0 * p.c_len, (const uint8_t*)nullptr,
                   (const uint8_t*)nullptr, (const uint8_t*)nullptr, (uint8_t*)nullptr, (int32_t*)nullptr, (size_t)0);
        }
    }
}
template <int K, int ETA1, int DU, int DV>
inline void decaps_shared_run(stream_t st, const ParamSet& p, size_t n, const uint8_t* dk, const uint8_t* c, uint8_t* Kout,
                              int32_t* status, const Workspace& ws) {
    constexpr int CLEN = 32 * (DU * K + DV);
    const Workspace& w = ws;
    if (status) {
        launch("k_hash_batch", k_hash_batch<0>, (size_t)1, WAVE, st, (size_t)1, dk + 384 * K, (unsigned)p.ek_len, (size_t)p.dk_len, ws.rho);
        launch("k_status_fill", k_status_fill, min_sz(ceil_div(n, 256), 1024), 256u, st, n, (const uint8_t*)ws.rho, dk + 768 * K + 32, status);
    }
    launch_sample_split(st, p, 1, 0, dk + 768 * K, p.dk_len, 1, nullptr, 0, 0, w);
    for (size_t h0 = 0; h0 < n; h0 += ws.hcap) {
        const size_t hn = min_sz(ws.hcap, n - h0);
        const uint8_t* ch = c + h0 * p.c_len;
        decrypt_launch<K, DU, DV>(st, hn, dk, (size_t)0, ch, ws.m);
        const size_t hgrid = ceil_div(hn, WAVE);
        if (!ws.fips)
            launch("k_hash_decaps", k_hash_decaps<K, CLEN, false, 168>, hgrid, WAVE, st, hn, dk, ch, (const uint8_t*)ws.m, ws.Kp, ws.r, ws.Kbar, (int32_t*)nullptr, (size_t)0);
        else
            launch("k_hash_decaps", k_hash_decaps<K, CLEN, false, 136>, hgrid, WAVE, st, hn, dk, ch, (const uint8_t*)ws.m, ws.Kp, ws.r, ws.Kbar, (int32_t*)nullptr, (size_t)0);
        for (size_t c0 = 0; c0 < hn; c0 += ws.cap) {
            const size_t cn = min_sz(ws.cap, hn - c0), i0 = h0 + c0;
            launch_sample_split(st, p, 0, cn, nullptr, 0, 1, ws.r + c0 * 32, 2 * K + 1, K, w);
            encrypt_launch<K, ETA1, DU, DV, true>("k_encrypt_cmp", st, cn, dk + 384 * K,
                   (size_t)0, (const uint8_t*)(ws.m + c0 * 32), (const uint16_t*)w.A, (const uint8_t*)w.prf, (uint8_t*)nullptr, c + i0 * p.c_len,
                   (const uint8_t*)(ws.Kp + c0 * 32), (const uint8_t*)(ws.Kbar + c0 * 32), Kout + i0 * 32, (int32_t*)nullptr, (size_t)0);
        }
    }
}
inline int encaps_shared_dispatch(stream_t st, int set, size_t n, const uint8_t* ek, const uint8_t* m, uint8_t* c, uint8_t* K, const Workspace& ws) {
    ParamSet p;
    if (!param_set(set, p)) return -1;
    if (n == 0) return 0;
    switch (set) {
    case 512: encaps_shared_run<2, 3, 10, 4>(st, p, n, ek, m, c, K, ws); break;
    case 768: encaps_shared_run<3, 2, 10, 4>(st, p, n, ek, m, c, K, ws); break;
    default: encaps_shared_run<4, 2, 11, 5>(st, p, n, ek, m, c, K, ws); break;
    }
    return 0;
}
inline int decaps_shared_dispatch(stream_t st, int set, size_t n, const uint8_t* dk, const uint8_t* c, uint8_t* K, int32_t* status,
                                  const Workspace& ws) {
    ParamSet p;
    if (!param_set(set, p)) return -1;
    if (n == 0) return 0;
    switch (set) {
    case 512: decaps_shared_run<2, 3, 10, 4>(st, p, n, dk, c, K, status, ws); break;
    case 768: decaps_shared_run<3, 2, 10, 4>(st, p, n, dk, c, K, status, ws); break;
    default: decaps_shared_run<4, 2, 11, 5>(st, p, n, dk, c, K, status, ws); break;
    }
    return 0;
}

inline int keygen_dispatch(stream_t st, int set, size_t n, const uint8_t* d, const uint8_t* z, uint8_t* ek, uint8_t* dk,
                           const Workspace& ws) {
    ParamSet p;
    if (!param_set(set, p)) return -1;
    switch (set) {
    case 512: keygen_run<2, 3>(st, p, n, d, z, ek, dk, ws); break;
    case 768: keygen_run<3, 2>(st, p, n, d, z, ek, dk, ws); break;
    default: keygen_run<4, 2>(st, p, n, d, z, ek, dk, ws); break;
    }
    return 0;
}
inline int encaps_dispatch(stream_t st, int set, size_t n, const uint8_t* ek, const uint8_t* m, uint8_t* c, uint8_t* K,
                           int32_t* mod_status, const Workspace& ws) {
    ParamSet p;
    if (!param_set(set, p)) return -1;
    switch (set) {
    case 512: encaps_run<2, 3, 10, 4>(st, p, n, ek, m, c, K, mod_status, ws); break;
    case 768: encaps_run<3, 2, 10, 4>(st, p, n, ek, m, c, K, mod_status, ws); break;
    default: encaps_run<4, 2, 11, 5>(st, p, n, ek, m, c, K, mod_status, ws); break;
    }
    return 0;
}
inline int pke_keygen_dispatch(stream_t st, int set, size_t n, const uint8_t* d, uint8_t* ek, uint8_t* dk_pke, const Workspace& ws) {
    return keygen_dispatch(st, set, n, d, nullptr, ek, dk_pke, ws);
}
inline int pke_encrypt_dispatch(stream_t st, int set, size_t n, const uint8_t* ek, const uint8_t* m, const uint8_t* r, uint8_t* c,
                                const Workspace& ws) {
    ParamSet p;
    if (!param_set(set, p) || !r) return -1;
    switch (set) {
    case 512: encaps_run<2, 3, 10, 4>(st, p, n, ek, m, c, nullptr, nullptr, ws, r); break;
    case 768: encaps_run<3, 2, 10, 4>(st, p, n, ek, m, c, nullptr, nullptr, ws, r); break;
    default: encaps_run<4, 2, 11, 5>(st, p, n, ek, m, c, nullptr, nullptr, ws, r); break;
    }
    return 0;
}
inline int pke_decrypt_dispatch(stream_t st, int set, size_t n, const uint8_t* dk_pke, const uint8_t* c, uint8_t* m) {
    ParamSet p;
    if (!param_set(set, p)) return -1;
    if (n == 0) return 0;
    switch (set) {
    case 512: decrypt_launch<2, 10, 4>(st, n, dk_pke, (size_t)(384 * 2), c, m); break;
    case 768: decrypt_launch<3, 10, 4>(st, n, dk_pke, (size_t)(384 * 3), c, m); break;
    default: decrypt_launch<4, 11, 5>(st, n, dk_pke, (size_t)(384 * 4), c, m); break;
    }
    return 0;
}
inline int decaps_dispatch(stream_t st, int set, size_t n, const uint8_t* dk, const uint8_t* c, uint8_t* K, int32_t* status,
                           bool hash_check, const Workspace& ws) {
    ParamSet p;
    if (!param_set(set, p)) return -1;
    switch (set) {
    case 512: decaps_run<2, 3, 10, 4>(st, p, n, dk, c, K, status, hash_check, ws); break;
    case 768: decaps_run<3, 2, 10, 4>(st, p, n, dk, c, K, status, hash_check, ws); break;
    default: decaps_run<4, 2, 11, 5>(st, p, n, dk, c, K, status, hash_check, ws); break;
    }
    return 0;
}

inline int decaps_seed_dispatch(stream_t st, int set, size_t n, const uint8_t* seed, const uint8_t* c, uint8_t* K, uint8_t* stage,
                                size_t stage_items, const Workspace& ws) {
    ParamSet p;
    if (!param_set(set, p)) return -1;
    switch (set) {
    case 512: decaps_seed_run<2, 3, 10, 4>(st, p, n, seed, c, K, stage, stage_items, ws); break;
    case 768: decaps_seed_run<3, 2, 10, 4>(st, p, n, seed, c, K, stage, stage_items, ws); break;
    default: decaps_seed_run<4, 2, 11, 5>(st, p, n, seed, c, K, stage, stage_items, ws); break;
    }
    return 0;
}

inline int check_keys_dispatch(stream_t st, int set, size_t n, const uint8_t* ek, const uint8_t* dk, const uint8_t* seed, const uint8_t* m,
                               int32_t* status, uint8_t* stage, size_t chunk, const Workspace& ws) {
    ParamSet p;
    if (!param_set(set, p)) return -1;
    switch (set) {
    case 512: check_keys_run<2, 3, 10, 4>(st, p, n, ek, dk, seed, m, status, stage, chunk, ws); break;
    case 768: check_keys_run<3, 2, 10, 4>(st, p, n, ek, dk, seed, m, status, stage, chunk, ws); break;
    default: check_keys_run<4, 2, 11, 5>(st, p, n, ek, dk, seed, m, status, stage, chunk, ws); break;
    }
    return 0;
}

inline size_t poly_grid(size_t n) {
    size_t g = ceil_div(n, ARITH_WAVES);
    const size_t cap = 256 * 16;
    return g < cap ? g : cap;
}
inline size_t ntt_grid_cap() {
    static const size_t v = [] {
        const char* e = getenv("MLKEM_NTT_GRID");
        const long long x = e ? atoll(e) : 0;
        return x > 0 ? (size_t)x : (size_t)(256 * 48);
    }();
    return v;
}
inline void ntt_launch(stream_t st, bool inverse, size_t n, const uint16_t* in, uint16_t* out) {
    size_t grid = ceil_div(ceil_div(n, 4), RNTT_WAVES);
    const size_t cap = ntt_grid_cap();
    if (grid > cap) grid = cap;
    if (inverse) launch("k_intt_batch", k_ntt4_batch<true>, grid, WAVE * RNTT_WAVES, st, n, in, out);
    else launch("k_ntt_batch", k_ntt4_batch<false>, grid, WAVE * RNTT_WAVES, st, n, in, out);
}
inline void basemul_launch(stream_t st, size_t n, const uint16_t* a, const uint16_t* b, uint16_t* h) {
    launch("k_basemul_batch", k_basemul_batch, poly_grid(n), WAVE * ARITH_WAVES, st, n, a, b, h);
}
inline int vecmul_launch(stream_t st, int k, size_t n, const uint16_t* u, const uint16_t* v, uint16_t* w) {
    if (k < 1 || k > 4) return -1;
    launch("k_vecmul_batch", k_vecmul_batch, poly_grid(n), WAVE * ARITH_WAVES, st, n, k, u, v, w);
    return 0;
}
inline void poly_addsub_launch(stream_t st, bool sub, size_t n_values, const uint16_t* a, const uint16_t* b, uint16_t* out) {
    size_t grid = ceil_div(ceil_div(n_values, 8), 256);
    if (grid > 256 * 8) grid = 256 * 8;
    if (sub) launch("k_poly_sub", k_poly_addsub<true>, grid, 256u, st, n_values, a, b, out);
    else launch("k_poly_add", k_poly_addsub<false>, grid, 256u, st, n_values, a, b, out);
}
inline int cbd_launch(stream_t st, int eta, size_t n, const uint8_t* bytes, uint16_t* out) {
    if (eta == 2) launch("k_cbd_batch", k_cbd_batch<2>, poly_grid(n), WAVE * ARITH_WAVES, st, n, bytes, out);
    else if (eta == 3) launch("k_cbd_batch", k_cbd_batch<3>, poly_grid(n), WAVE * ARITH_WAVES, st, n, bytes, out);
    else return -1;
    return 0;
}
inline int codec_launch(stream_t st, bool encode, int d, size_t n, const void* in, void* out) {
#define MLKEM_CODEC_CASE(D)                                                                                                    \
    case D:                                                                                                                    \
        if (encode) launch("k_encode_batch", k_encode_batch<D>, poly_grid(n), WAVE * ARITH_WAVES, st, n, (const uint16_t*)in, (uint8_t*)out); \
        else launch("k_decode_batch", k_decode_batch<D>, poly_grid(n), WAVE * ARITH_WAVES, st, n, (const uint8_t*)in, (uint16_t*)out);        \
        return 0;
    switch (d) {
        MLKEM_CODEC_CASE(1) MLKEM_CODEC_CASE(4) MLKEM_CODEC_CASE(5) MLKEM_CODEC_CASE(10) MLKEM_CODEC_CASE(11) MLKEM_CODEC_CASE(12)
    default: return -1;
    }
#undef MLKEM_CODEC_CASE
}
inline int compress_values_launch(stream_t st, bool decompress, int d, size_t n, const uint16_t* in, uint16_t* out) {
    if (d < 1 || d > 12) return -1;
    size_t grid = ceil_div(ceil_div(n, 8), 256);
    if (grid > 256 * 8) grid = 256 * 8;
    if (grid == 0) return 0;
    if (decompress) launch("k_decompress_values", k_compress_values<true>, grid, 256u, st, n, d, in, out);
    else launch("k_compress_values", k_compress_values<false>, grid, 256u, st, n, d, in, out);
    return 0;
}
template <int QB = KQ, int CAP = SAMPLE_CAP>
inline void sample_ntt_launch(stream_t st, size_t n, const uint8_t* seeds34, uint16_t* out, size_t wave_max = 0, uint8_t* retries = nullptr) {
    if (n <= wave_max) {
        launch("k_sample_xof", k_sample_ntt_w<QB, CAP>, n, WAVE, st, n, seeds34, out, retries);
        return;
    }
    SampleArgs a{};
    a.n_xof = n; a.rho = seeds34; a.rho_stride = 34; a.K = 0; a.A = out; a.retries = retries;
    a.xof_blocks = (unsigned)ceil_div(n, WAVE);
    launch("k_sample_xof", k_sample<QB, CAP>, (size_t)a.xof_blocks, WAVE, st, a);
}
inline int prf_launch(stream_t st, int eta, size_t n, const uint8_t* in33, uint8_t* out) {
    if (eta != 2 && eta != 3) return -1;
    SampleArgs a{};
    a.n_prf = n; a.r = in33; a.per_item = 0; a.eta1 = eta; a.prf = out; a.prf_stride = 64u * (unsigned)eta;
    launch("k_sample_prf", k_sample<>, ceil_div(n, WAVE), WAVE, st, a);
    return 0;
}
inline int hash_launch(stream_t st, int kind, size_t n, const uint8_t* msg, unsigned len, size_t stride, uint8_t* out) {
    if (kind < 0 || kind > 2 || (stride & 7) || stride < len) return -1;
    const size_t grid = ceil_div(n, WAVE);
    if (kind == 0) launch("k_hash_batch", k_hash_batch<0>, grid, WAVE, st, n, msg, len, stride, out);
    else if (kind == 1) launch("k_hash_batch", k_hash_batch<1>, grid, WAVE, st, n, msg, len, stride, out);
    else launch("k_hash_batch", k_hash_batch<2>, grid, WAVE, st, n, msg, len, stride, out);
    return 0;
}

inline void cells_launch(stream_t st, bool to_bytes, size_t n, const void* in, void* out) {
    size_t grid = ceil_div(ceil_div(n, 16), 256);
    if (grid > 256 * 8) grid = 256 * 8;
    if (grid == 0) grid = 1;
    if (to_bytes) launch("k_cells_to_bytes", k_cells_to_bytes, grid, 256u, st, n, (const uint32_t*)in, (uint8_t*)out);
    else launch("k_bytes_to_cells", k_bytes_to_cells, grid, 256u, st, n, (const uint8_t*)in, (uint32_t*)out);
}

inline int sponge_raw_launch(stream_t st, unsigned rate, size_t n, const uint8_t* msg, unsigned nblocks, uint8_t* out, unsigned outlen,
                             size_t out_stride, size_t wave_max = 0) {
    if (nblocks == 0 || out_stride < outlen || rate == 0 || rate >= 200) return -1;
    const bool standard = rate == 72 || rate == 104 || rate == 136 || rate == 144 || rate == 168;
    if (n <= wave_max || !standard) {
        launch("k_sponge_raw", k_sponge_raw_w, n, WAVE, st, n, msg, rate, nblocks, out, outlen, out_stride);
        return 0;
    }
    if (out_stride & 3) return -1;
    const size_t grid = ceil_div(n, WAVE);
    switch (rate) {
    case 72: launch("k_sponge_raw", k_sponge_raw<72>, grid, WAVE, st, n, msg, nblocks, out, outlen, out_stride); break;
    case 104: launch("k_sponge_raw", k_sponge_raw<104>, grid, WAVE, st, n, msg, nblocks, out, outlen, out_stride); break;
    case 136: launch("k_sponge_raw", k_sponge_raw<136>, grid, WAVE, st, n, msg, nblocks, out, outlen, out_stride); break;
    case 144: launch("k_sponge_raw", k_sponge_raw<144>, grid, WAVE, st, n, msg, nblocks, out, outlen, out_stride); break;
    case 168: launch("k_sponge_raw", k_sponge_raw<168>, grid, WAVE, st, n, msg, nblocks, out, outlen, out_stride); break;
    default: return -1;
    }
    return 0;
}

inline int sha3_ragged_launch(stream_t st, unsigned rate, const Sha3rArgs& a, size_t wave_max) {
    if (a.n <= wave_max) {
        launch("k_sha3_ragged", k_sha3_ragged_w, a.n, WAVE, st, a, rate);
        return 0;
    }
    const size_t grid = ceil_div(a.n, WAVE);
    switch (rate) {
    case 72: launch("k_sha3_ragged", k_sha3_ragged<72>, grid, WAVE, st, a); break;
    case 104: launch("k_sha3_ragged", k_sha3_ragged<104>, grid, WAVE, st, a); break;
    case 136: launch("k_sha3_ragged", k_sha3_ragged<136>, grid, WAVE, st, a); break;
    case 144: launch("k_sha3_ragged", k_sha3_ragged<144>, grid, WAVE, st, a); break;
    case 168: launch("k_sha3_ragged", k_sha3_ragged<168>, grid, WAVE, st, a); break;
    default: return -1;
    }
    return 0;
}

}
```

Baseline: 62.34 million.

## Defer implicit-rejection J hash to only items whose re-encryption mismatches

Decapsulation previously computed Kbar = J(z||c) for every item, absorbing the full ciphertext through a sponge, and blended it with K' after the re-encrypt compare. Now the compare kernel writes K' (masked to zero on reject) and appends rejected item indices to an atomic list. A separate kernel then hashes J only for the listed items. For valid ciphertexts this removes a full ciphertext read and the Keccak permutations, at the cost of an extra reset and launch plus an atomic per rejected item.

Result: faster. 65.51 million, median of 6 (+5.1%).

```diff
diff --git a/crystals-kyber_amd/csrc/mlkem_kernels.hpp b/crystals-kyber_amd/csrc/mlkem_kernels.hpp
--- a/crystals-kyber_amd/csrc/mlkem_kernels.hpp
+++ b/crystals-kyber_amd/csrc/mlkem_kernels.hpp
@@ -314,12 +314,11 @@
     else z[2 * item + part - 2] = v;
 }
 
-template <int K, int CLEN, bool HASH_CHECK, int JRATE = 168>
-__global__ void __launch_bounds__(WAVE, MLKEM_KECCAK_MINWAVES) k_hash_decaps(size_t n, const uint8_t* __restrict__ dk, const uint8_t* __restrict__ c,
-                                                      const uint8_t* __restrict__ m_ws, uint8_t* __restrict__ Kp_ws,
-                                                      uint8_t* __restrict__ r_ws, uint8_t* __restrict__ Kbar_ws,
-                                                      int32_t* __restrict__ status, size_t dk_stride) {
-    __shared__ __attribute__((aligned(16))) uint2 stage[STAGE_QWORDS];
+template <int K, bool HASH_CHECK>
+__global__ void __launch_bounds__(WAVE, MLKEM_KECCAK_MINWAVES) k_hash_decaps(size_t n, const uint8_t* __restrict__ dk, const uint8_t* __restrict__ m_ws,
+                                                      uint8_t* __restrict__ Kp_ws, uint8_t* __restrict__ r_ws, int32_t* __restrict__ status,
+                                                      size_t dk_stride) {
+    __shared__ __attribute__((aligned(16))) uint2 stage[HASH_CHECK ? stage_qwords(136) : 1];
     constexpr unsigned EK = 384 * K + 32;
     const size_t DK = dk_stride;
     const size_t nb = (n + WAVE - 1) / WAVE;
@@ -343,15 +342,6 @@
         if (i2 < n && status) status[i2] = diff ? -5 : 0;
         return;
     }
-    {
-        MsgView mv{dk + 768 * K + 64, DK, 32, c, CLEN, CLEN};
-        wave_sponge_absorb<JRATE, 0x1F>(s, stage, mv, item0, n);
-        const size_t i2 = item0 + (size_t)lane_id_fresh();
-        if (i2 < n) {
-            MLKEM_STATE_WORDS8(s, 0, w)
-            store32(Kbar_ws, 32, i2, w);
-        }
-    }
     uint32_t mm[8];
     const size_t it = my_item();
     load32(m_ws, 32, it, mm);
@@ -364,6 +354,77 @@
         MLKEM_STATE_WORDS8(s, 8, w)
         store32(r_ws, 32, item, w);
         if (!HASH_CHECK && status) status[item] = 0;
+    }
+}
+
+constexpr int REJ_HDR = 4;
+constexpr int CMP_NONE = 0, CMP_BLEND = 1, CMP_DEFER = 2;
+constexpr int J_GROUP = 8;
+
+__device__ __forceinline__ size_t keyset_key(const uint32_t* __restrict__ idx, size_t n_keys, size_t item) {
+    if (!idx) return 0;
+    const size_t k = idx[item];
+    return k < n_keys ? k : 0;
+}
+
+template <int CLEN, int JRATE>
+__global__ void __launch_bounds__(WAVE, MLKEM_KECCAK_MINWAVES) k_hash_j_rejected(const uint32_t* __restrict__ list, size_t hn,
+                                                                                 const uint8_t* __restrict__ z, size_t z_stride,
+                                                                                 const uint32_t* __restrict__ idx, size_t n_keys,
+                                                                                 const uint8_t* __restrict__ c, uint8_t* __restrict__ Kout) {
+    constexpr int NQ = JRATE / 8;
+    constexpr unsigned TOTAL = 32u + (unsigned)CLEN, NFULL = TOTAL / (unsigned)JRATE, REM = TOTAL % (unsigned)JRATE;
+    static_assert(CLEN % 8 == 0 && JRATE % 8 == 0, "qword absorb");
+    const uint32_t hn32 = (uint32_t)hn, cnt = list[0] < hn32 ? list[0] : hn32;
+    for (uint32_t base = blockIdx.x * (uint32_t)WAVE; base < cnt; base += gridDim.x * (uint32_t)WAVE) {
+        auto my_item = [&]() {
+            const uint32_t slot = base + (uint32_t)lane_id_fresh();
+            const uint32_t it = list[REJ_HDR + (slot < cnt - 1u ? slot : cnt - 1u)];
+            return (size_t)(it < hn32 - 1u ? it : hn32 - 1u);
+        };
+        KeccakState s;
+        keccak_zero(s);
+#pragma unroll 1
+        for (unsigned b = 0; b <= NFULL; b++) {
+            const unsigned pos0 = b * (unsigned)JRATE;
+            const size_t it = my_item();
+            const uint8_t *zb = z, *cbase = c;
+#ifndef MLKEM_EMU
+            asm volatile("" : "+s"(zb), "+s"(cbase));
+#endif
+            const uint8_t* zr = zb + (n_keys ? keyset_key(idx, n_keys, it) : it) * z_stride;
+            const uint8_t* cb = cbase + it * (size_t)CLEN + pos0;
+#pragma unroll
+            for (int w0 = 0; w0 < NQ; w0 += J_GROUP) {
+                uint2 raw[J_GROUP];
+#pragma unroll
+                for (int k = 0; k < J_GROUP; k++) {
+                    const int w = w0 + k;
+                    raw[k].x = 0; raw[k].y = 0;
+                    const uint8_t* src = cb + (8 * w - 32);
+                    if (w < 4) src = b == 0 ? zr + 8 * w : src;
+                    if (w < NQ && pos0 + 8u * (unsigned)w < TOTAL) raw[k] = *reinterpret_cast<const uint2*>(src);
+                }
+#pragma unroll
+                for (int k = 0; k < J_GROUP; k++) {
+                    if (w0 + k >= NQ) break;
+                    s.lo[w0 + k] ^= raw[k].x;
+                    s.hi[w0 + k] ^= raw[k].y;
+                }
+                pin_state<NQ>(s);
+                sched_fence();
+            }
+            const bool last = b == NFULL;
+            keccak_xor_byte<REM>(s, last ? 0x1Fu : 0u);
+            keccak_xor_byte<JRATE - 1>(s, last ? 0x80u : 0u);
+            keccak_f1600(s);
+        }
+        const uint32_t slot = base + (uint32_t)lane_id_fresh();
+        if (slot < cnt) {
+            uint32_t w[8];
+            MLKEM_STATE_WORDS8(s, 0, w)
+            store32(Kout, 32, my_item(), w);
+        }
     }
 }
 
diff --git a/crystals-kyber_amd/csrc/mlkem_keyset.hpp b/crystals-kyber_amd/csrc/mlkem_keyset.hpp
--- a/crystals-kyber_amd/csrc/mlkem_keyset.hpp
+++ b/crystals-kyber_amd/csrc/mlkem_keyset.hpp
@@ -30,11 +30,6 @@
     }
 };
 
-__device__ __forceinline__ size_t keyset_key(const uint32_t* __restrict__ idx, size_t n_keys, size_t item) {
-    if (!idx) return 0;
-    const size_t k = idx[item];
-    return k < n_keys ? k : 0;
-}
 
 __global__ void __launch_bounds__(WAVE, MLKEM_KECCAK_MINWAVES) k_hash_g_keyset(size_t n, const uint32_t* __restrict__ idx, size_t n_keys,
                                                                                const uint8_t* __restrict__ m, const uint8_t* __restrict__ hs,
@@ -54,63 +49,42 @@
     }
 }
 
-__global__ void __launch_bounds__(256) k_keyset_gather32(size_t n, const uint32_t* __restrict__ idx, size_t n_keys, const uint8_t* __restrict__ src,
-                                                         size_t stride, uint32_t* __restrict__ dst) {
-    const size_t g = (size_t)blockIdx.x * blockDim.x + threadIdx.x;
-    if (g >= 8 * n) return;
-    const size_t item = g >> 3;
-    dst[g] = reinterpret_cast<const uint32_t*>(src + keyset_key(idx, n_keys, item) * stride)[g & 7];
-}
-
-template <int K, int CLEN, int JRATE>
 __global__ void __launch_bounds__(WAVE, MLKEM_KECCAK_MINWAVES) k_hash_decaps_keyset(size_t n, const uint32_t* __restrict__ idx, size_t n_keys,
-                                                                                    const uint8_t* __restrict__ hs, uint8_t* __restrict__ z_ws,
-                                                                                    const uint8_t* __restrict__ c, const uint8_t* __restrict__ m_ws,
-                                                                                    uint8_t* __restrict__ Kp_ws, uint8_t* __restrict__ r_ws,
-                                                                                    uint8_t* __restrict__ Kbar_ws) {
-    __shared__ __attribute__((aligned(16))) uint2 stage[STAGE_QWORDS];
-    const size_t item0 = (size_t)blockIdx.x * WAVE;
+                                                                                    const uint8_t* __restrict__ hs, uint8_t* __restrict__ zero_ws,
+                                                                                    const uint8_t* __restrict__ m_ws, uint8_t* __restrict__ Kp_ws,
+                                                                                    uint8_t* __restrict__ r_ws) {
+    const size_t item = (size_t)blockIdx.x * WAVE + lane_id();
+    const size_t it = item < n ? item : n - 1;
+    uint32_t mm[8], hh[8], w[8];
+    load32(m_ws, 32, it, mm);
+    load32(hs, 32, keyset_key(idx, n_keys, it), hh);
     KeccakState s;
-    uint32_t h[8], w[8];
-    {
-        MsgView mv{z_ws, 32, 32, c, CLEN, CLEN};
-        wave_sponge_absorb<JRATE, 0x1F>(s, stage, mv, item0, n);
-        const size_t i2 = item0 + (size_t)lane_id_fresh();
-        if (i2 < n) {
-            MLKEM_STATE_WORDS8(s, 0, w)
-            store32(Kbar_ws, 32, i2, w);
-            uint32_t* zr = reinterpret_cast<uint32_t*>(z_ws + i2 * 32);
-#pragma unroll
-            for (int q = 0; q < 8; q++) zr[q] = 0u;
-        }
-    }
-    uint32_t mm[8];
-    const size_t i3 = item0 + (size_t)lane_id_fresh(), it = i3 < n ? i3 : n - 1;
-    load32(m_ws, 32, it, mm);
-    load32(hs, 32, keyset_key(idx, n_keys, it), h);
-    lane_G64(s, mm, h);
-    const size_t item = item0 + (size_t)lane_id_fresh();
+    lane_G64(s, mm, hh);
     if (item < n) {
         MLKEM_STATE_WORDS8(s, 0, w)
         store32(Kp_ws, 32, item, w);
         MLKEM_STATE_WORDS8(s, 8, w)
         store32(r_ws, 32, item, w);
-    }
-}
-
-template <int K, int ETA1, int DU, int DV, bool COMPARE>
+#pragma unroll
+        for (int q = 0; q < 8; q++) w[q] = 0u;
+        store32(zero_ws, 32, item, w);
+    }
+}
+
+template <int K, int ETA1, int DU, int DV, int CMP>
 __global__ void __launch_bounds__(WAVE * KPKE2_WAVES, kpke2_minwaves(K))
 k_encrypt2_keyset(size_t n, const uint32_t* __restrict__ idx, size_t n_keys, const uint8_t* __restrict__ ek, size_t ek_stride,
                   const uint16_t* __restrict__ At, const uint8_t* __restrict__ msg, const uint8_t* __restrict__ prf, uint8_t* __restrict__ c_out,
-                  const uint8_t* __restrict__ c_in, const uint8_t* __restrict__ Kp, const uint8_t* __restrict__ Kbar, uint8_t* __restrict__ Kout) {
+                  const uint8_t* __restrict__ c_in, const uint8_t* __restrict__ Kp, uint8_t* __restrict__ Kout, uint32_t* __restrict__ rej,
+                  uint32_t rej_base) {
     __shared__ K2Lds<K + 1> lds_all[KPKE2_WAVES];
     const int wv = wave_id();
     const size_t item0 = 2 * ((size_t)blockIdx.x * KPKE2_WAVES + wv);
     if (item0 >= n) return;
     const size_t h = (size_t)(lane_id() >> 5), item = item0 + h < n ? item0 + h : item0;
     const size_t key = keyset_key(idx, n_keys, item);
-    encrypt2_body<K, ETA1, DU, DV, COMPARE>(lds_all[wv].xch, item0, n, ek + key * ek_stride, 0, msg, At + key * (size_t)(K * K * 256), prf,
-                                            c_out, c_in, Kp, Kbar, Kout, (int32_t*)nullptr, 0);
+    encrypt2_body<K, ETA1, DU, DV, CMP>(lds_all[wv].xch, item0, n, ek + key * ek_stride, 0, msg, At + key * (size_t)(K * K * 256), prf,
+                                        c_out, c_in, Kp, (const uint8_t*)nullptr, Kout, (int32_t*)nullptr, 0, rej, rej_base);
 }
 
 template <int K, int DU, int DV>
@@ -329,9 +303,9 @@
         for (size_t c0 = 0; c0 < hn; c0 += ws.cap) {
             const size_t cn = min_sz(ws.cap, hn - c0), i0 = h0 + c0;
             launch_sample_split(st, p, 0, cn, nullptr, 0, 1, ws.r + c0 * 32, 2 * K + 1, K, ws);
-            launch("k_encrypt_keyset", k_encrypt2_keyset<K, ETA1, DU, DV, false>, ceil_div(ceil_div(cn, 2), KPKE2_WAVES), WAVE * KPKE2_WAVES, st, cn,
+            launch("k_encrypt_keyset", k_encrypt2_keyset<K, ETA1, DU, DV, CMP_NONE>, ceil_div(ceil_div(cn, 2), KPKE2_WAVES), WAVE * KPKE2_WAVES, st, cn,
                    idx ? idx + i0 : nullptr, ks.n_keys, ek, ks.key_stride, ks.At, m + i0 * 32, (const uint8_t*)ws.prf, c + i0 * p.c_len,
-                   (const uint8_t*)nullptr, (const uint8_t*)nullptr, (const uint8_t*)nullptr, (uint8_t*)nullptr);
+                   (const uint8_t*)nullptr, (const uint8_t*)nullptr, (uint8_t*)nullptr, (uint32_t*)nullptr, 0u);
         }
     }
     if (idx || status)
@@ -360,22 +334,18 @@
         const uint8_t* ch = c + h0 * p.c_len;
         launch("k_decrypt_keyset", k_decrypt4_keyset<K, DU, DV>, ceil_div(ceil_div(hn, 4), KPKE4_WAVES), 64 * KPKE4_WAVES, st, hn, idh, ks.n_keys,
                ks.keys, ks.key_stride, ch, ws.m);
-        launch("k_keyset_gather32", k_keyset_gather32, ceil_div(8 * hn, 256), 256u, st, hn, idh, ks.n_keys, ks.keys + 768 * K + 64, ks.key_stride,
-               reinterpret_cast<uint32_t*>(ws.rho));
-        if (!ws.fips)
-            launch("k_hash_decaps_keyset", k_hash_decaps_keyset<K, CLEN, 168>, ceil_div(hn, WAVE), WAVE, st, hn, idh, ks.n_keys, ks.h,
-                   ws.rho, ch, (const uint8_t*)ws.m, ws.Kp, ws.r, ws.Kbar);
-        else
-            launch("k_hash_decaps_keyset", k_hash_decaps_keyset<K, CLEN, 136>, ceil_div(hn, WAVE), WAVE, st, hn, idh, ks.n_keys, ks.h,
-                   ws.rho, ch, (const uint8_t*)ws.m, ws.Kp, ws.r, ws.Kbar);
+        reject_list_reset(st, ws);
+        launch("k_hash_decaps_keyset", k_hash_decaps_keyset, ceil_div(hn, WAVE), WAVE, st, hn, idh, ks.n_keys, ks.h, ws.rho, (const uint8_t*)ws.m,
+               ws.Kp, ws.r);
         for (size_t c0 = 0; c0 < hn; c0 += ws.cap) {
             const size_t cn = min_sz(ws.cap, hn - c0), i0 = h0 + c0;
             launch_sample_split(st, p, 0, cn, nullptr, 0, 1, ws.r + c0 * 32, 2 * K + 1, K, ws);
-            launch("k_encrypt_cmp_keyset", k_encrypt2_keyset<K, ETA1, DU, DV, true>, ceil_div(ceil_div(cn, 2), KPKE2_WAVES), WAVE * KPKE2_WAVES, st,
-                   cn, idx ? idx + i0 : nullptr, ks.n_keys, ks.keys + 384 * K, ks.key_stride, ks.At, (const uint8_t*)(ws.m + c0 * 32),
-                   (const uint8_t*)ws.prf, (uint8_t*)nullptr, c + i0 * p.c_len, (const uint8_t*)(ws.Kp + c0 * 32), (const uint8_t*)(ws.Kbar + c0 * 32),
-                   Kout + i0 * 32);
+            launch("k_encrypt_cmp_keyset", k_encrypt2_keyset<K, ETA1, DU, DV, CMP_DEFER>, ceil_div(ceil_div(cn, 2), KPKE2_WAVES), WAVE * KPKE2_WAVES,
+                   st, cn, idx ? idx + i0 : nullptr, ks.n_keys, ks.keys + 384 * K, ks.key_stride, ks.At, (const uint8_t*)(ws.m + c0 * 32),
+                   (const uint8_t*)ws.prf, (uint8_t*)nullptr, c + i0 * p.c_len, (const uint8_t*)(ws.Kp + c0 * 32), Kout + i0 * 32, reject_list(ws),
+                   (uint32_t)c0);
         }
+        j_rejected_launch<CLEN>(st, ws, hn, ks.keys + 768 * K + 64, ks.key_stride, idh, ks.n_keys, ch, Kout + h0 * 32);
     }
     if (idx || status)
         launch("k_keyset_fix", k_keyset_fix, min_sz(ceil_div(n, 256), 1024), 256u, st, n, idx, ks.n_keys, (uint8_t*)nullptr, p.c_len, Kout, status);
diff --git a/crystals-kyber_amd/csrc/mlkem_kpke2.hpp b/crystals-kyber_amd/csrc/mlkem_kpke2.hpp
--- a/crystals-kyber_amd/csrc/mlkem_kpke2.hpp
+++ b/crystals-kyber_amd/csrc/mlkem_kpke2.hpp
@@ -406,12 +406,13 @@
     return 0;
 }
 
-template <int K, int ETA1, int DU, int DV, bool COMPARE>
+template <int K, int ETA1, int DU, int DV, int CMP>
 __device__ __forceinline__ void
 encrypt2_body(float2 (*xch)[2][128], size_t item0, size_t n, const uint8_t* __restrict__ ek, size_t ek_stride, const uint8_t* __restrict__ msg,
               const uint16_t* __restrict__ A, const uint8_t* __restrict__ prf, uint8_t* __restrict__ c_out, const uint8_t* __restrict__ c_in,
               const uint8_t* __restrict__ Kp, const uint8_t* __restrict__ Kbar, uint8_t* __restrict__ Kout, int32_t* __restrict__ mod_status,
-              size_t a_stride) {
+              size_t a_stride, uint32_t* __restrict__ rej = nullptr, uint32_t rej_base = 0) {
+    constexpr bool COMPARE = CMP != CMP_NONE;
     const int l = lane_id(), h = l >> 5, t = l & 31, nb = k2_blk(t);
     const bool valid = item0 + (size_t)h < n;
     const unsigned hh = valid ? (unsigned)h : 0u;
@@ -510,13 +511,25 @@
         const bool bad = ((bal >> (32 * h)) & 0xFFFFFFFFull) != 0;
         if (t == 0 && valid) mod_status[item] = bad ? -4 : 0;
     }
-    if constexpr (COMPARE) {
+    if constexpr (CMP == CMP_BLEND) {
         const unsigned long long bal = __ballot(diff != 0);
         const uint32_t reject = ((bal >> (32 * h)) & 0xFFFFFFFFull) != 0 ? 0xFFFFFFFFu : 0u;
         if (t < 8 && valid) {
             const uint32_t kp = reinterpret_cast<const uint32_t*>(Kp + item * 32)[t];
             const uint32_t kb = reinterpret_cast<const uint32_t*>(Kbar + item * 32)[t];
             reinterpret_cast<uint32_t*>(Kout + item * 32)[t] = (kp & ~reject) | (kb & reject);
+        }
+    }
+    if constexpr (CMP == CMP_DEFER) {
+        const unsigned long long bal = __ballot(diff != 0);
+        const uint32_t reject = ((bal >> (32 * h)) & 0xFFFFFFFFull) != 0 ? 0xFFFFFFFFu : 0u;
+        if (t < 8 && valid) {
+            const uint32_t kp = reinterpret_cast<const uint32_t*>(Kp + item * 32)[t];
+            reinterpret_cast<uint32_t*>(Kout + item * 32)[t] = kp & ~reject;
+        }
+        if (t == 0 && valid && reject) {
+            const uint32_t j = atomicAdd(&rej[0], 1u);
+            rej[REJ_HDR + j] = rej_base + (uint32_t)item;
         }
     }
 }
@@ -637,16 +650,18 @@
     }
 }
 
-template <int K, int ETA1, int DU, int DV, bool COMPARE>
+template <int K, int ETA1, int DU, int DV, int CMP>
 __global__ void __launch_bounds__(WAVE * KPKE2_WAVES, kpke2_minwaves(K))
 k_encrypt2(size_t n, const uint8_t* __restrict__ ek, size_t ek_stride, const uint8_t* __restrict__ msg, const uint16_t* __restrict__ A,
            const uint8_t* __restrict__ prf, uint8_t* __restrict__ c_out, const uint8_t* __restrict__ c_in, const uint8_t* __restrict__ Kp,
-           const uint8_t* __restrict__ Kbar, uint8_t* __restrict__ Kout, int32_t* __restrict__ mod_status, size_t a_stride) {
+           const uint8_t* __restrict__ Kbar, uint8_t* __restrict__ Kout, int32_t* __restrict__ mod_status, size_t a_stride,
+           uint32_t* __restrict__ rej, uint32_t rej_base) {
     __shared__ K2Lds<K + 1> lds_all[KPKE2_WAVES];
     const int wv = wave_id();
     const size_t item0 = 2 * ((size_t)blockIdx.x * KPKE2_WAVES + wv);
     if (item0 >= n) return;
-    encrypt2_body<K, ETA1, DU, DV, COMPARE>(lds_all[wv].xch, item0, n, ek, ek_stride, msg, A, prf, c_out, c_in, Kp, Kbar, Kout, mod_status, a_stride);
+    encrypt2_body<K, ETA1, DU, DV, CMP>(lds_all[wv].xch, item0, n, ek, ek_stride, msg, A, prf, c_out, c_in, Kp, Kbar, Kout, mod_status, a_stride,
+                                        rej, rej_base);
 }
 
 __device__ __forceinline__ void k2_canon(const v2f (&p)[4], unsigned (&c)[8]) {
diff --git a/crystals-kyber_amd/csrc/mlkem_pipeline.hpp b/crystals-kyber_amd/csrc/mlkem_pipeline.hpp
--- a/crystals-kyber_amd/csrc/mlkem_pipeline.hpp
+++ b/crystals-kyber_amd/csrc/mlkem_pipeline.hpp
@@ -175,9 +175,22 @@
     launch_sample_split<QB, CAP>(st, p, n, n, rho, rho_stride, transpose, r, prf_per_item, n_eta1, ws);
 }
 
-template <int K, int ETA1, int DU, int DV, bool CMP, class... Args>
+template <int K, int ETA1, int DU, int DV, int CMP, class... Args>
 inline void encrypt_launch(const char* label, stream_t st, size_t n, Args... args) {
     launch(label, k_encrypt2<K, ETA1, DU, DV, CMP>, ceil_div(ceil_div(n, 2), KPKE2_WAVES), WAVE * KPKE2_WAVES, st, n, args...);
+}
+
+inline uint32_t* reject_list(const Workspace& ws) { return reinterpret_cast<uint32_t*>(ws.Kbar); }
+inline void reject_list_reset(stream_t st, const Workspace& ws) { zero_u32x2(st, reject_list(ws)); }
+template <int CLEN>
+inline void j_rejected_launch(stream_t st, const Workspace& ws, size_t hn, const uint8_t* z, size_t z_stride, const uint32_t* idx, size_t n_keys,
+                              const uint8_t* ch, uint8_t* Kh) {
+    if (!(ws.stages & 1u)) return;
+    const size_t grid = min_sz(ceil_div(hn, WAVE), 2048);
+    if (!ws.fips)
+        launch("k_hash_j_rejected", k_hash_j_rejected<CLEN, 168>, grid, WAVE, st, (const uint32_t*)reject_list(ws), hn, z, z_stride, idx, n_keys, ch, Kh);
+    else
+        launch("k_hash_j_rejected", k_hash_j_rejected<CLEN, 136>, grid, WAVE, st, (const uint32_t*)reject_list(ws), hn, z, z_stride, idx, n_keys, ch, Kh);
 }
 
 template <int K, int ETA1>
@@ -250,9 +263,9 @@
                 launch_sample(st, p, cn, eki + 384 * K, p.ek_len, 1, r_h + c0 * 32, 2 * K + 1, K, ws);
             }
             if (ws.stages & 4u)
-            encrypt_launch<K, ETA1, DU, DV, false>("k_encrypt", st, cn, eki, (size_t)p.ek_len, m + i0 * 32, (const uint16_t*)ws.A, (const uint8_t*)ws.prf,
+            encrypt_launch<K, ETA1, DU, DV, CMP_NONE>("k_encrypt", st, cn, eki, (size_t)p.ek_len, m + i0 * 32, (const uint16_t*)ws.A, (const uint8_t*)ws.prf,
                    c + i0 * p.c_len, (const uint8_t*)nullptr, (const uint8_t*)nullptr, (const uint8_t*)nullptr, (uint8_t*)nullptr,
-                   mod_status ? mod_status + i0 : (int32_t*)nullptr, (size_t)(K * K * 256));
+                   mod_status ? mod_status + i0 : (int32_t*)nullptr, (size_t)(K * K * 256), (uint32_t*)nullptr, 0u);
         }
     }
 }
@@ -289,8 +302,10 @@
         if (ws.stages & 8u) decrypt_launch<K, DU, DV>(st, hn, dkh, (size_t)p.dk_len, ch, ws.m);
         int32_t* sth = (hash_check && status) ? status + h0 : (int32_t*)nullptr;
         const size_t hgrid = ceil_div(hn, WAVE);
+        const bool wide = n <= ws.wide_kem(K);
+        if (!wide) reject_list_reset(st, ws);
         if (!(ws.stages & 1u)) {
-        } else if (n <= ws.wide_kem(K)) {
+        } else if (wide) {
             if (hash_check && !ws.fips)
                 launch("k_hash_decaps", k_hash_decaps_w<K, CLEN, true, 168>, 2 * hn, WAVE, st, hn, dkh, ch, (const uint8_t*)ws.m, ws.Kp, ws.r, ws.Kbar, sth, (size_t)p.dk_len);
             else if (!ws.fips)
@@ -299,15 +314,10 @@
                 launch("k_hash_decaps", k_hash_decaps_w<K, CLEN, true, 136>, 2 * hn, WAVE, st, hn, dkh, ch, (const uint8_t*)ws.m, ws.Kp, ws.r, ws.Kbar, sth, (size_t)p.dk_len);
             else
                 launch("k_hash_decaps", k_hash_decaps_w<K, CLEN, false, 136>, hn, WAVE, st, hn, dkh, ch, (const uint8_t*)ws.m, ws.Kp, ws.r, ws.Kbar, sth, (size_t)p.dk_len);
-        } else
-        if (hash_check && !ws.fips)
-            launch("k_hash_decaps", k_hash_decaps<K, CLEN, true, 168>, 2 * hgrid, WAVE, st, hn, dkh, ch, (const uint8_t*)ws.m, ws.Kp, ws.r, ws.Kbar, sth, (size_t)p.dk_len);
-        else if (!ws.fips)
-            launch("k_hash_decaps", k_hash_decaps<K, CLEN, false, 168>, hgrid, WAVE, st, hn, dkh, ch, (const uint8_t*)ws.m, ws.Kp, ws.r, ws.Kbar, sth, (size_t)p.dk_len);
-        else if (hash_check)
-            launch("k_hash_decaps", k_hash_decaps<K, CLEN, true, 136>, 2 * hgrid, WAVE, st, hn, dkh, ch, (const uint8_t*)ws.m, ws.Kp, ws.r, ws.Kbar, sth, (size_t)p.dk_len);
+        } else if (hash_check)
+            launch("k_hash_decaps", k_hash_decaps<K, true>, 2 * hgrid, WAVE, st, hn, dkh, (const uint8_t*)ws.m, ws.Kp, ws.r, sth, (size_t)p.dk_len);
         else
-            launch("k_hash_decaps", k_hash_decaps<K, CLEN, false, 136>, hgrid, WAVE, st, hn, dkh, ch, (const uint8_t*)ws.m, ws.Kp, ws.r, ws.Kbar, sth, (size_t)p.dk_len);
+            launch("k_hash_decaps", k_hash_decaps<K, false>, hgrid, WAVE, st, hn, dkh, (const uint8_t*)ws.m, ws.Kp, ws.r, sth, (size_t)p.dk_len);
         for (size_t c0 = 0; c0 < hn; c0 += ws.cap) {
             const size_t cn = min_sz(ws.cap, hn - c0), i0 = h0 + c0;
             const uint8_t* dki = dk + i0 * p.dk_len;
@@ -317,11 +327,17 @@
             } else if (ws.stages & 2u) {
                 launch_sample(st, p, cn, dki + 768 * K, p.dk_len, 1, ws.r + c0 * 32, 2 * K + 1, K, ws);
             }
-            if (ws.stages & 4u)
-            encrypt_launch<K, ETA1, DU, DV, true>("k_encrypt_cmp", st, cn, dki + 384 * K, (size_t)p.dk_len, (const uint8_t*)(ws.m + c0 * 32), (const uint16_t*)ws.A,
-                   (const uint8_t*)ws.prf, (uint8_t*)nullptr, c + i0 * p.c_len, (const uint8_t*)(ws.Kp + c0 * 32),
-                   (const uint8_t*)(ws.Kbar + c0 * 32), Kout + i0 * 32, (int32_t*)nullptr, (size_t)(K * K * 256));
-        }
+            if (!(ws.stages & 4u)) continue;
+            if (wide)
+                encrypt_launch<K, ETA1, DU, DV, CMP_BLEND>("k_encrypt_cmp", st, cn, dki + 384 * K, (size_t)p.dk_len, (const uint8_t*)(ws.m + c0 * 32),
+                       (const uint16_t*)ws.A, (const uint8_t*)ws.prf, (uint8_t*)nullptr, c + i0 * p.c_len, (const uint8_t*)(ws.Kp + c0 * 32),
+                       (const uint8_t*)(ws.Kbar + c0 * 32), Kout + i0 * 32, (int32_t*)nullptr, (size_t)(K * K * 256), (uint32_t*)nullptr, 0u);
+            else
+                encrypt_launch<K, ETA1, DU, DV, CMP_DEFER>("k_encrypt_cmp", st, cn, dki + 384 * K, (size_t)p.dk_len, (const uint8_t*)(ws.m + c0 * 32),
+                       (const uint16_t*)ws.A, (const uint8_t*)ws.prf, (uint8_t*)nullptr, c + i0 * p.c_len, (const uint8_t*)(ws.Kp + c0 * 32),
+                       (const uint8_t*)nullptr, Kout + i0 * 32, (int32_t*)nullptr, (size_t)(K * K * 256), reject_list(ws), (uint32_t)c0);
+        }
+        if (!wide) j_rejected_launch<CLEN>(st, ws, hn, dkh + 768 * K + 64, (size_t)p.dk_len, (const uint32_t*)nullptr, (size_t)0, ch, Kout + h0 * 32);
     }
 }
 
@@ -417,9 +433,9 @@
         for (size_t c0 = 0; c0 < hn; c0 += ws.cap) {
             const size_t cn = min_sz(ws.cap, hn - c0), i0 = h0 + c0;
             launch_sample_split(st, p, 0, cn, nullptr, 0, 1, ws.r + c0 * 32, 2 * K + 1, K, w);
-            encrypt_launch<K, ETA1, DU, DV, false>("k_encrypt", st, cn, ek, (size_t)0,
+            encrypt_launch<K, ETA1, DU, DV, CMP_NONE>("k_encrypt", st, cn, ek, (size_t)0,
                    m + i0 * 32, (const uint16_t*)w.A, (const uint8_t*)w.prf, c + i0 * p.c_len, (const uint8_t*)nullptr,
-                   (const uint8_t*)nullptr, (const uint8_t*)nullptr, (uint8_t*)nullptr, (int32_t*)nullptr, (size_t)0);
+                   (const uint8_t*)nullptr, (const uint8_t*)nullptr, (uint8_t*)nullptr, (int32_t*)nullptr, (size_t)0, (uint32_t*)nullptr, 0u);
         }
     }
 }
@@ -438,17 +454,17 @@
         const uint8_t* ch = c + h0 * p.c_len;
         decrypt_launch<K, DU, DV>(st, hn, dk, (size_t)0, ch, ws.m);
         const size_t hgrid = ceil_div(hn, WAVE);
-        if (!ws.fips)
-            launch("k_hash_decaps", k_hash_decaps<K, CLEN, false, 168>, hgrid, WAVE, st, hn, dk, ch, (const uint8_t*)ws.m, ws.Kp, ws.r, ws.Kbar, (int32_t*)nullptr, (size_t)0);
-        else
-            launch("k_hash_decaps", k_hash_decaps<K, CLEN, false, 136>, hgrid, WAVE, st, hn, dk, ch, (const uint8_t*)ws.m, ws.Kp, ws.r, ws.Kbar, (int32_t*)nullptr, (size_t)0);
+        reject_list_reset(st, ws);
+        launch("k_hash_decaps", k_hash_decaps<K, false>, hgrid, WAVE, st, hn, dk, (const uint8_t*)ws.m, ws.Kp, ws.r, (int32_t*)nullptr, (size_t)0);
         for (size_t c0 = 0; c0 < hn; c0 += ws.cap) {
             const size_t cn = min_sz(ws.cap, hn - c0), i0 = h0 + c0;
             launch_sample_split(st, p, 0, cn, nullptr, 0, 1, ws.r + c0 * 32, 2 * K + 1, K, w);
-            encrypt_launch<K, ETA1, DU, DV, true>("k_encrypt_cmp", st, cn, dk + 384 * K,
+            encrypt_launch<K, ETA1, DU, DV, CMP_DEFER>("k_encrypt_cmp", st, cn, dk + 384 * K,
                    (size_t)0, (const uint8_t*)(ws.m + c0 * 32), (const uint16_t*)w.A, (const uint8_t*)w.prf, (uint8_t*)nullptr, c + i0 * p.c_len,
-                   (const uint8_t*)(ws.Kp + c0 * 32), (const uint8_t*)(ws.Kbar + c0 * 32), Kout + i0 * 32, (int32_t*)nullptr, (size_t)0);
-        }
+                   (const uint8_t*)(ws.Kp + c0 * 32), (const uint8_t*)nullptr, Kout + i0 * 32, (int32_t*)nullptr, (size_t)0, reject_list(ws),
+                   (uint32_t)c0);
+        }
+        j_rejected_launch<CLEN>(st, ws, hn, dk + 768 * K + 64, (size_t)0, (const uint32_t*)nullptr, (size_t)0, ch, Kout + h0 * 32);
     }
 }
 inline int encaps_shared_dispatch(stream_t st, int set, size_t n, const uint8_t* ek, const uint8_t* m, uint8_t* c, uint8_t* K, const Workspace& ws) {
```
